# AgentCooper2002/AudioDiffuser

Measured on AMD Instinct MI355X. Metric: audio samples/sec (16384-sample waveform, 50-step Heun), higher is better.
Workload: dtype bf16; 1 GPU; BASELINE configs[1]: UNet1d 64 ch (c2), 16384-sample waveforms, KarrasSchedule N=50 heun, batch 64/GPU, random-init weights; global_batch=64, sampler=heun, num_steps=50, nfe=99, hipgraph=True, parallelism=batch-sharded x1, one all-gather

## Files before the change

### audiodiffuser_amd/_lib.py

```python
from __future__ import annotations

import ctypes as C
import os
from typing import Optional

from .config import UNet1dConfig

HERE = os.path.dirname(os.path.abspath(__file__))
LIB_PATH = os.environ.get("ADF_HIP_LIB") or os.path.join(HERE, "libadf_hip.so")
ADF_MAX_LAYERS = 12
DTYPE_F32, DTYPE_BF16, DTYPE_F32X3 = 0, 1, 2
FLAG_SEPARATE_GN_STATS = 1
SAMPLER_EDM, SAMPLER_EDM_ALPHA, SAMPLER_DPM_MULTISTEP, SAMPLER_DPM2, SAMPLER_ADPM2 = 0, 1, 2, 3, 4
SAMPLER_LMS, SAMPLER_DPM_SINGLESTEP, SAMPLER_DPM2M, SAMPLER_UNIPC, SAMPLER_ADPMPP2S = 5, 6, 7, 8, 9
SAMPLER_RF_EULER = 10


class AdfNetConfig(C.Structure):
    _fields_ = [
        ("channels", C.c_int32), ("num_filters", C.c_int32), ("window_length", C.c_int32), ("stride", C.c_int32),
        ("in_channels", C.c_int32), ("out_channels", C.c_int32),
        ("resnet_groups", C.c_int32), ("kernel_multiplier_downsample", C.c_int32),
        ("num_layers", C.c_int32),
        ("multipliers", C.c_int32 * (ADF_MAX_LAYERS + 1)),
        ("factors", C.c_int32 * ADF_MAX_LAYERS),
        ("num_blocks", C.c_int32 * ADF_MAX_LAYERS),
        ("attentions", C.c_int32 * ADF_MAX_LAYERS),
        ("attention_heads", C.c_int32), ("attention_multiplier", C.c_int32),
        ("use_skip_scale", C.c_int32), ("use_attention_bottleneck", C.c_int32),
        ("dtype", C.c_int32), ("flags", C.c_int32), ("num_classes", C.c_int32),
    ]


class AdfSamplerDesc(C.Structure):
    _fields_ = [
        ("kind", C.c_int32), ("num_steps", C.c_int32),
        ("s_tmin", C.c_float), ("s_tmax", C.c_float), ("s_churn", C.c_float), ("s_noise", C.c_float),
        ("use_heun", C.c_int32), ("alpha", C.c_float), ("order", C.c_int32), ("sigma_data", C.c_float),
        ("use_graph", C.c_int32), ("rho", C.c_float), ("eta", C.c_float), ("log_time_spacing", C.c_int32), ("eps_pred", C.c_int32),
        ("reflow", C.c_int32),
    ]


def make_sampler_desc(kind: int, num_steps: int, sigma_data: float, use_graph: bool, **fields) -> AdfSamplerDesc:
    unknown = set(fields) - {name for name, _ in AdfSamplerDesc._fields_}
    if unknown:
        raise TypeError(f"adf_sampler_desc has no field {sorted(unknown)}")
    return AdfSamplerDesc(kind=kind, num_steps=int(num_steps), sigma_data=sigma_data, use_graph=int(use_graph),
                          **{"s_noise": 1.0, "alpha": 1.0, **fields})


class AdfWaveNetConfig(C.Structure):
    _fields_ = [("residual_channels", C.c_int32), ("residual_layers", C.c_int32), ("dilation_cycle", C.c_int32),
                ("dim_in", C.c_int32), ("dim_mid", C.c_int32), ("dim_out", C.c_int32), ("dtype", C.c_int32)]


ADF_ADM_MAX_LEVELS = 8


class AdfAdmConfig(C.Structure):
    _fields_ = [("in_channels", C.c_int32), ("model_channels", C.c_int32), ("out_channels", C.c_int32), ("num_res_blocks", C.c_int32),
                ("n_mult", C.c_int32), ("channel_mult", C.c_int32 * ADF_ADM_MAX_LEVELS),
                ("n_attention_ds", C.c_int32), ("attention_ds", C.c_int32 * ADF_ADM_MAX_LEVELS),
                ("conv_resample", C.c_int32), ("num_heads", C.c_int32), ("num_head_channels", C.c_int32), ("use_scale_shift_norm", C.c_int32),
                ("resblock_updown", C.c_int32), ("use_new_attention_order", C.c_int32), ("num_classes", C.c_int32), ("dtype", C.c_int32)]


ADF_U2D_MAX_LEVELS, ADF_U2D_MAX_INIT_KERNELS = 8, 4


class AdfUNet2dConfig(C.Structure):
    _fields_ = [("ff_mult", C.c_double),
                ("dim", C.c_int32), ("cond_dim", C.c_int32), ("channels", C.c_int32), ("channels_out", C.c_int32), ("num_classes", C.c_int32),
                ("n_levels", C.c_int32), ("dim_mults", C.c_int32 * ADF_U2D_MAX_LEVELS),
                ("layer_attns", C.c_int32 * ADF_U2D_MAX_LEVELS), ("layer_cross_attns", C.c_int32 * ADF_U2D_MAX_LEVELS),
                ("num_resnet_blocks", C.c_int32), ("resnet_groups", C.c_int32), ("attn_heads", C.c_int32),
                ("layer_attns_depth", C.c_int32), ("layer_mid_attns_depth", C.c_int32), ("attend_at_middle", C.c_int32),
                ("n_init_kernels", C.c_int32), ("init_kernel_sizes", C.c_int32 * ADF_U2D_MAX_INIT_KERNELS),
                ("learned_sinu_pos_emb_dim", C.c_int32), ("num_time_tokens", C.c_int32),
                ("scale_skip_connection", C.c_int32), ("final_resnet_block", C.c_int32), ("dtype", C.c_int32)]


class AdfRunCounters(C.Structure):
    _fields_ = [("sampler_runs", C.c_int64), ("sampler_evals", C.c_int64), ("graph_captures", C.c_int64),
                ("graph_replays", C.c_int64), ("denoise_calls", C.c_int64), ("net_passes", C.c_int64)]


class AdfIstftConfig(C.Structure):
    _fields_ = [("n_fft", C.c_int32), ("hop_length", C.c_int32), ("center", C.c_int32), ("normalized", C.c_int32),
                ("spec_abs_exponent", C.c_double), ("spec_factor", C.c_double)]


FLAG_NEAREST_UPSAMPLE = 2
PRECOND_EDM, PRECOND_VE, PRECOND_VP, PRECOND_V_EDM = 0, 1, 2, 3
PRECOND_RF, PRECOND_RF_EDM = 4, 5
LOSS_X0_EDM, LOSS_X0_INV_SIGMA2, LOSS_RF = 0, 1, 2
LOSS_CHUNK = 4096
ABI_VERSION = 7

EXPORTS = {
    "adf_abi_version": (C.c_int, []),
    "adf_get_counters": (C.c_int, [C.c_void_p, C.POINTER(AdfRunCounters)]),
    "adf_create": (C.c_int, [C.POINTER(AdfNetConfig), C.POINTER(C.c_void_p)]),
    "adf_wavenet_create": (C.c_int, [C.POINTER(AdfWaveNetConfig), C.POINTER(C.c_void_p)]),
    "adf_adm_create": (C.c_int, [C.POINTER(AdfAdmConfig), C.POINTER(C.c_void_p)]),
    "adf_unet2d_create": (C.c_int, [C.POINTER(AdfUNet2dConfig), C.POINTER(C.c_void_p)]),
    "adf_set_image_shape": (C.c_int, [C.c_void_p, C.c_int, C.c_int]),
    "adf_set_dynamic_threshold": (C.c_int, [C.c_void_p, C.c_float]),
    "adf_set_preconditioning": (C.c_int, [C.c_void_p, C.c_int, C.c_double, C.c_double, C.c_double]),
    "adf_debug_coef_rows": (C.c_int, [C.c_void_p, C.c_void_p, C.c_int, C.POINTER(C.c_int), C.c_void_p]),
    "adf_destroy": (None, [C.c_void_p]),
    "adf_last_error": (C.c_char_p, [C.c_void_p]),
    "adf_num_weights": (C.c_int, [C.c_void_p]),
    "adf_weight_name": (C.c_char_p, [C.c_void_p, C.c_int]),
    "adf_weight_numel": (C.c_int64, [C.c_void_p, C.c_int]),
    "adf_load_weight": (C.c_int, [C.c_void_p, C.c_char_p, C.c_void_p, C.c_int64, C.c_void_p]),
    "adf_weights_missing": (C.c_int, [C.c_void_p]),
    "adf_set_condition": (C.c_int, [C.c_void_p, C.c_void_p, C.c_int, C.c_int, C.c_float, C.c_void_p]),
    "adf_net_forward": (C.c_int, [C.c_void_p, C.c_void_p, C.c_void_p, C.c_void_p, C.c_int, C.c_int, C.c_void_p]),
    "adf_denoise": (C.c_int, [C.c_void_p, C.c_void_p, C.c_void_p, C.c_float, C.c_float, C.c_void_p, C.c_int, C.c_int, C.c_void_p]),
    "adf_sampler_run": (C.c_int, [C.c_void_p, C.POINTER(AdfSamplerDesc), C.POINTER(C.c_float), C.c_int, C.c_void_p,
                                  C.c_void_p, C.c_int, C.c_void_p, C.c_int, C.c_int, C.c_void_p]),
    "adf_diffusion_loss": (C.c_int, [C.c_void_p, C.c_int, C.c_void_p, C.c_void_p, C.c_void_p, C.c_float, C.c_void_p, C.c_void_p, C.c_void_p,
                                     C.c_int, C.c_int, C.c_void_p]),
    "adf_loss_calls": (C.c_int64, [C.c_void_p]),
    "adf_sampler_nfe": (C.c_int, [C.POINTER(AdfSamplerDesc), C.POINTER(C.c_float), C.c_int]),
    "adf_debug_tap_shape": (C.c_int, [C.c_void_p, C.c_char_p, C.POINTER(C.c_int), C.POINTER(C.c_int)]),
    "adf_debug_tap_copy": (C.c_int, [C.c_void_p, C.c_char_p, C.c_void_p, C.c_void_p]),
    "adf_debug_tap_stats": (C.c_int, [C.c_void_p, C.c_char_p, C.c_void_p, C.POINTER(C.c_int), C.c_void_p]),
    "adf_debug_up_tile_plan": (C.c_int, [C.c_int, C.c_int, C.c_int, C.c_int, C.c_int, C.POINTER(C.c_int), C.POINTER(C.c_int), C.POINTER(C.c_int),
                                         C.POINTER(C.c_int)]),
    "adf_debug_dyn_threshold": (C.c_int, [C.c_void_p, C.c_void_p, C.c_int, C.c_longlong, C.c_float, C.c_void_p]),
    "adf_debug_tap_count": (C.c_int, [C.c_void_p]),
    "adf_debug_tap_name": (C.c_char_p, [C.c_void_p, C.c_int]),
    "adf_device_bytes": (C.c_int64, [C.c_void_p]),
    "adf_bench_resblock": (C.c_int, [C.c_void_p, C.c_int, C.c_int, C.c_int, C.c_int, C.POINTER(C.c_float), C.POINTER(C.c_float),
                                     C.POINTER(C.c_double), C.POINTER(C.c_double), C.POINTER(C.c_double), C.POINTER(C.c_double),
                                     C.c_void_p]),
    "adf_bench_layer": (C.c_int, [C.c_void_p, C.c_int, C.c_int, C.c_int, C.c_int, C.c_int, C.POINTER(C.c_float), C.POINTER(C.c_double),
                                  C.POINTER(C.c_double), C.POINTER(C.c_int), C.c_void_p]),
    "adf_bench_wavenet_layer": (C.c_int, [C.c_void_p, C.c_int, C.c_int, C.c_int, C.c_int, C.POINTER(C.c_float), C.POINTER(C.c_double),
                                          C.POINTER(C.c_double), C.c_void_p]),
    "adf_bench_loss_kernels": (C.c_int, [C.c_void_p, C.c_int, C.c_int, C.c_longlong, C.c_int, C.POINTER(C.c_float), C.POINTER(C.c_float),
                                         C.POINTER(C.c_double), C.POINTER(C.c_double), C.c_void_p]),
    "adf_istft_create": (C.c_int, [C.POINTER(AdfIstftConfig), C.c_void_p, C.POINTER(C.c_void_p)]),
    "adf_istft_basis": (C.c_int, [C.POINTER(AdfIstftConfig), C.c_void_p, C.c_void_p, C.c_void_p]),
    "adf_istft_run": (C.c_int, [C.c_void_p, C.c_void_p, C.c_int, C.c_int, C.c_void_p, C.c_int64, C.c_void_p]),
    "adf_istft_destroy": (None, [C.c_void_p]),
    "adf_stft_create": (C.c_int, [C.POINTER(AdfIstftConfig), C.c_void_p, C.POINTER(C.c_void_p)]),
    "adf_stft_basis": (C.c_int, [C.POINTER(AdfIstftConfig), C.c_void_p, C.c_void_p]),
    "adf_stft_run": (C.c_int, [C.c_void_p, C.c_void_p, C.c_int, C.c_int64, C.c_void_p, C.c_int, C.c_void_p]),
    "adf_stft_destroy": (None, [C.c_void_p]),
}

_lib: Optional[C.CDLL] = None


def load_library() -> C.CDLL:
    global _lib
    if _lib is not None:
        return _lib
    if not os.path.exists(LIB_PATH):
        raise RuntimeError(
            f"{LIB_PATH} is missing: build it with `python -m audiodiffuser_amd.build` "
            "(or __graft_entry__.build()). There is no CPU/PyTorch fallback for the HIP path.")
    lib = C.CDLL(LIB_PATH)
    for name, (res, args) in EXPORTS.items():
        fn = getattr(lib, name)
        fn.restype = res
        fn.argtypes = args
    got = lib.adf_abi_version()
    if got != ABI_VERSION:
        raise RuntimeError(f"{LIB_PATH} reports ABI version {got}, this binding was written against {ABI_VERSION}: rebuild the "
                           "library (python -m audiodiffuser_amd.build --force)")
    _lib = lib
    return lib


def make_config(cfg: UNet1dConfig, dtype: int, flags: int = 0) -> AdfNetConfig:
    cfg.validate()
    n = cfg.num_layers
    if n > ADF_MAX_LAYERS:
        raise ValueError("too many layers")
    c = AdfNetConfig()
    c.channels, c.num_filters, c.window_length, c.stride = cfg.channels, cfg.num_filters, cfg.window_length, cfg.stride
    c.in_channels, c.out_channels = cfg.in_channels, cfg.out_channels
    c.resnet_groups, c.kernel_multiplier_downsample = cfg.resnet_groups, cfg.kernel_multiplier_downsample
    c.num_layers = n
    for i, m in enumerate(cfg.multipliers):
        c.multipliers[i] = int(m)
    for i in range(n):
        c.factors[i] = int(cfg.factors[i])
        c.num_blocks[i] = int(cfg.num_blocks[i])
        c.attentions[i] = 1 if cfg.attentions[i] else 0
    c.attention_heads, c.attention_multiplier = cfg.attention_heads, cfg.attention_multiplier
    c.use_skip_scale = 1 if cfg.use_skip_scale else 0
    c.use_attention_bottleneck = 1 if cfg.use_attention_bottleneck else 0
    c.dtype, c.flags = dtype, flags | (FLAG_NEAREST_UPSAMPLE if cfg.use_nearest_upsample else 0)
    c.num_classes = int(cfg.num_classes) if cfg.class_cond else 0
    return c


def make_adm_config(cfg, dtype: int) -> AdfAdmConfig:
    c = AdfAdmConfig()
    c.in_channels, c.model_channels, c.out_channels, c.num_res_blocks = cfg.in_channels, cfg.model_channels, cfg.out_channels, cfg.num_res_blocks
    if len(cfg.channel_mult) > ADF_ADM_MAX_LEVELS or len(cfg.attention_ds) > ADF_ADM_MAX_LEVELS:
        raise ValueError("too many levels")
    c.n_mult = len(cfg.channel_mult)
    for i, m in enumerate(cfg.channel_mult):
        if int(m) != m:
            raise ValueError("channel_mult entries must be integers")
        c.channel_mult[i] = int(m)
    c.n_attention_ds = len(cfg.attention_ds)
    for i, d in enumerate(cfg.attention_ds):
        c.attention_ds[i] = int(d)
    c.conv_resample, c.num_heads, c.num_head_channels = int(cfg.conv_resample), cfg.num_heads, cfg.num_head_channels
    c.use_scale_shift_norm, c.resblock_updown = int(cfg.use_scale_shift_norm), int(cfg.resblock_updown)
    c.use_new_attention_order = int(cfg.use_new_attention_order)
    c.num_classes = int(cfg.num_classes) if cfg.num_classes is not None else 0
    c.dtype = dtype
    return c


def make_unet2d_config(cfg, dtype: int) -> AdfUNet2dConfig:
    n = len(cfg.dim_mults)
    if n > ADF_U2D_MAX_LEVELS or len(cfg.init_cross_embed_kernel_sizes) > ADF_U2D_MAX_INIT_KERNELS:
        raise ValueError("too many levels / cross-embed kernel sizes")
    c = AdfUNet2dConfig()
    c.ff_mult = float(cfg.ff_mult)
    c.dim, c.cond_dim, c.channels, c.channels_out, c.num_classes = cfg.dim, cfg.cdim, cfg.channels, cfg.out_channels, int(cfg.num_classes)
    c.n_levels = n
    for i in range(n):
        c.dim_mults[i], c.layer_attns[i], c.layer_cross_attns[i] = int(cfg.dim_mults[i]), int(cfg.layer_attns[i]), int(cfg.layer_cross_attns[i])
    c.num_resnet_blocks, c.resnet_groups, c.attn_heads = cfg.num_resnet_blocks, cfg.resnet_groups, cfg.attn_heads
    c.layer_attns_depth, c.layer_mid_attns_depth, c.attend_at_middle = cfg.layer_attns_depth, cfg.layer_mid_attns_depth, int(cfg.attend_at_middle)
    ks = sorted(cfg.init_cross_embed_kernel_sizes)
    c.n_init_kernels = len(ks)
    for i, k in enumerate(ks):
        c.init_kernel_sizes[i] = int(k)
    c.learned_sinu_pos_emb_dim, c.num_time_tokens = cfg.learned_sinu_pos_emb_dim, cfg.num_time_tokens
    c.scale_skip_connection, c.final_resnet_block = int(cfg.scale_skip_connection), int(cfg.final_resnet_block)
    c.dtype = dtype
    return c


def make_wavenet_config(cfg, dtype: int) -> AdfWaveNetConfig:
    c = AdfWaveNetConfig()
    c.residual_channels, c.residual_layers, c.dilation_cycle = cfg.residual_channels, cfg.residual_layers, cfg.dilation_cycle
    c.dim_in, c.dim_mid, c.dim_out = cfg.dim_in, cfg.dim_mid, cfg.dim_out
    c.dtype = dtype
    return c


class AdfError(RuntimeError):
    pass


def check(lib: C.CDLL, handle, rc: int, what: str) -> None:
    if rc != 0:
        msg = lib.adf_last_error(handle)
        raise AdfError(f"{what}: {msg.decode() if msg else 'unknown error'}")
```

### audiodiffuser_amd/csrc/adf_gemm.h

```cpp
#pragma once
#include "adf_common.h"

namespace adf {

constexpr int kARows = 144;
constexpr int kTapGroup = 3;

struct GemmSeg {
    const void* src0;
    const void* src1;
    int c0, c1;
    const float* ab;
    GnFinalizeArgs gn;
    float scale1;
    int act;
    int taps, stride, off0, step;
    const void* w;
    const void* wfrag;
    int nchunk;
};

struct GemmArgs {
    GemmSeg seg[2];
    int nseg;
    int B, lin, mrows, n, n_pad;
    int gn_ready;
    int flat;
    int seg_rows;
    const float* bias0;
    const float* bias1;
    int bias_mod;
    const void* res;
    int gelu;
    void* out;
    int out_rows, out_c;
    int scatter_f, scatter_pad;
    int phase_c;
    double* stats;
    int stats_groups;
};

template <int N>
__device__ __forceinline__ void gemm_bias_load(const GemmArgs& a, const int (&bi)[N], const bool (&ok)[N], float (&out)[N]) {
    const bool h0 = a.bias0 != nullptr, h1 = a.bias1 != nullptr;
    const float* const dmy = (const float*)a.seg[0].w;
    const float* const p0 = h0 ? a.bias0 : dmy;
    const float* const p1 = h1 ? a.bias1 : dmy;
    float v0[N], v1[N];
#pragma unroll
    for (int k = 0; k < N; ++k) {
        const int idx = ok[k] ? bi[k] : 0;
        v0[k] = p0[h0 ? idx : 0]; v1[k] = p1[h1 ? idx : 0];
    }
#pragma unroll
    for (int k = 0; k < N; ++k) out[k] = ok[k] ? (h0 ? v0[k] : 0.f) + (h1 ? v1[k] : 0.f) : 0.f;
}

typedef __attribute__((ext_vector_type(8))) __bf16 bf16x8_t;
typedef __attribute__((ext_vector_type(16))) float f32x16_t;
typedef __attribute__((ext_vector_type(4))) float f32x4_t;
typedef __attribute__((ext_vector_type(2))) float f32x2_t;


constexpr int kLdsPitch = 144;
__device__ __forceinline__ int lds_swz(int row, int c16) { return row * kLdsPitch + (c16 << 4); }

#define ADF_GLOAD16(dst, ptr) asm volatile("global_load_dwordx4 %0, %1, off" : "=v"(dst) : "v"(ptr) : "memory")

__device__ __forceinline__ const char* uniform_ptr(const void* p) {
    const unsigned long long v = (unsigned long long)p;
    const unsigned lo = __builtin_amdgcn_readfirstlane((unsigned)v);
    const unsigned hi = __builtin_amdgcn_readfirstlane((unsigned)(v >> 32));
    return (const char*)(((unsigned long long)hi << 32) | lo);
}

template <int TM, int TN>
constexpr int gemm_lds_bytes() {
    constexpr int main_b = kARows * kLdsPitch + kTapGroup * TN * kLdsPitch;
    constexpr int epi_b = TM * TN * 4;
    return main_b > epi_b ? main_b : epi_b;
}

template <int TAPS, int MT, int NT, typename FA, typename FW>
__device__ __forceinline__ void mfma_chunk_bf16(f32x16_t (&acc)[MT][NT], int h, FA addrA, FW addrW) {
    constexpr int NS = TAPS * 4;
    bf16x8_t fa[2][MT], fb[2][NT];
#pragma unroll
    for (int i = 0; i < MT; ++i) fa[0][i] = *(const bf16x8_t*)addrA(0, i, h);
#pragma unroll
    for (int j = 0; j < NT; ++j) fb[0][j] = *(const bf16x8_t*)addrW(0, j, h);
#pragma unroll
    for (int st = 0; st < NS; ++st) {
        const int cur = st & 1, nxt = cur ^ 1;
        if (st + 1 < NS) {
            const int tap = (st + 1) >> 2, ks = (st + 1) & 3;
#pragma unroll
            for (int i = 0; i < MT; ++i) fa[nxt][i] = *(const bf16x8_t*)addrA(tap, i, ks * 2 + h);
#pragma unroll
            for (int j = 0; j < NT; ++j) fb[nxt][j] = *(const bf16x8_t*)addrW(tap, j, ks * 2 + h);
        }
        __builtin_amdgcn_sched_barrier(0);
#pragma unroll
        for (int i = 0; i < MT; ++i)
#pragma unroll
            for (int j = 0; j < NT; ++j)
                acc[i][j] = __builtin_amdgcn_mfma_f32_32x32x16_bf16(fa[cur][i], fb[cur][j], acc[i][j], 0, 0, 0);
        __builtin_amdgcn_sched_barrier(0);
    }
}

template <typename T, int MT, int NT, int WM, int WN>
__global__ void __launch_bounds__(64 * WM * WN) conv_gemm_kernel(const GemmArgs a) {
    constexpr int TM = 32 * MT * WM, TN = 32 * NT * WN, NTHR = 64 * WM * WN;
    constexpr int EPC = Elem<T>::kPerChunk;
    constexpr int KC = kRowBytes / (int)sizeof(T);
    constexpr int A_CH = (kARows * 8 + NTHR - 1) / NTHR;
    constexpr int W_CH = (kTapGroup * TN * 8 + NTHR - 1) / NTHR;
    constexpr bool kBf16 = sizeof(T) == 2;
    constexpr bool kX3 = IsX3<T>::value;
    extern __shared__ __attribute__((aligned(16))) char smem[];
    char* ldsA = smem;
    char* ldsW = smem + kARows * kLdsPitch;

    const int tid = threadIdx.x, lane = tid & 63, wave = tid >> 6;
    const int r = lane & 31, h = lane >> 5;
    const int wm = wave / WN, wn = wave % WN;
    const int tiles_n = (a.n_pad + TN - 1) / TN;
    int bid = blockIdx.x;
    const int tn_i = bid % tiles_n; bid /= tiles_n;
    const int seg = a.flat ? a.seg_rows : TM;
    const int nsegs = TM / seg;
    int b0, m0;
    long long R0;
    if (a.flat) {
        R0 = (long long)bid * TM;
        b0 = (int)(R0 / a.mrows);
        m0 = 0;
    } else {
        const int tiles_m = (a.mrows + TM - 1) / TM;
        const int tm_i = bid % tiles_m;
        b0 = bid / tiles_m;
        m0 = tm_i * TM;
        R0 = (long long)b0 * a.mrows + m0;
    }
    const int n0 = tn_i * TN;
    const int c16 = tid & 7;

    f32x16_t acc[MT][NT];
#pragma unroll
    for (int i = 0; i < MT; ++i)
#pragma unroll
        for (int j = 0; j < NT; ++j)
#pragma unroll
            for (int e = 0; e < 16; ++e) acc[i][j][e] = 0.f;

    const int ntg0 = (a.seg[0].taps + kTapGroup - 1) / kTapGroup;
    const int nit0 = a.seg[0].nchunk * ntg0;
    const int ntg1 = a.nseg > 1 ? (a.seg[1].taps + kTapGroup - 1) / kTapGroup : 1;
    const int nit = nit0 + (a.nseg > 1 ? a.seg[1].nchunk * ntg1 : 0);

    u32x4_t ra[A_CH];
    u32x4_t rw[W_CH];
    f32x4_t abq[EPC / 2];
    float raw_scale = 1.0f;
    unsigned avalid = 0;

    const int wrow0 = tid >> 3;
    int arow_idx[A_CH];
    auto setup_segment = [&](const GemmSeg& sg) {
        const int off_min = sg.step > 0 ? sg.off0 : sg.off0 - (sg.taps - 1);
        const int segrows = (seg - 1) * sg.stride + sg.taps;
        const int nrows = nsegs * segrows;
        const int p_lo = m0 * sg.stride + off_min;
#pragma unroll
        for (int i = 0; i < A_CH; ++i) {
            const int row = (tid + i * NTHR) >> 3;
            const int j = a.flat ? row / segrows : 0;
            const int p = p_lo + (row - j * segrows);
            const int bb = b0 + j;
            const bool ok = row < nrows && p >= 0 && p < a.lin && bb < a.B;
            arow_idx[i] = ok ? bb * a.lin + p : -1;
        }
    };
    auto load_regs = [&](int it) {
        const bool s1 = it >= nit0;
        const GemmSeg& sg = s1 ? a.seg[1] : a.seg[0];
        const int local = s1 ? it - nit0 : it;
        const int ntg = s1 ? ntg1 : ntg0;
        const int chunk = local / ntg, tg = local - chunk * ntg;
        if (local == 0) setup_segment(sg);
        if (tg == 0) {
            const int ctot = sg.c0 + sg.c1;
            const int cidx = chunk * KC + c16 * EPC;
            const bool cvalid = cidx < ctot;
            const bool from1 = sg.c1 > 0 && cidx >= sg.c0;
            const char* src0u = uniform_ptr(sg.src0);
            const char* src1u = uniform_ptr(sg.src1);
            const char* src = from1 ? src1u : src0u;
            const int c0u = __builtin_amdgcn_readfirstlane(sg.c0), c1u = __builtin_amdgcn_readfirstlane(sg.c1);
            const unsigned rowbytes = (unsigned)(from1 ? c1u : c0u) * (unsigned)sizeof(T);
            const unsigned colbytes = (unsigned)(from1 ? cidx - c0u : cidx) * (unsigned)sizeof(T);
            avalid = 0;
#pragma unroll
            for (int i = 0; i < A_CH; ++i) {
                const bool ok = cvalid && arow_idx[i] >= 0;
                const unsigned off = ok ? (unsigned)arow_idx[i] * rowbytes + colbytes : 0u;
                ra[i] = *(const u32x4_t*)(src + off);
                avalid |= (ok ? 1u : 0u) << i;
            }
            const float* abp = sg.ab ? sg.ab + (cvalid ? (unsigned)(b0 * ctot + cidx) * 2u : 0u) : (const float*)sg.w;
#pragma unroll
            for (int e = 0; e < EPC / 2; ++e) abq[e] = *(const f32x4_t*)(abp + e * 4);
            raw_scale = from1 ? sg.scale1 : 1.0f;
        }
        const char* wp = (const char*)sg.w + (size_t)(chunk * sg.taps + tg * kTapGroup) * a.n_pad * kRowBytes;
#pragma unroll
        for (int i = 0; i < W_CH; ++i) {
            const int row = wrow0 + i * (NTHR / 8);
            const int tap_l = row / TN, n_l = row - tap_l * TN;
            const unsigned woff = (unsigned)((tap_l * a.n_pad + n0 + n_l) * kRowBytes + c16 * 16);
            rw[i] = *(const u32x4_t*)(wp + woff);
        }
    };

    const int lds_row0 = tid >> 3;
    auto store_lds = [&](int it) {
        const bool s1 = it >= nit0;
        const GemmSeg& sg = s1 ? a.seg[1] : a.seg[0];
        const int local = s1 ? it - nit0 : it;
        const int ntg = s1 ? ntg1 : ntg0;
        const int tg = local % ntg;
        if (tg == 0) {
            const int nrows = nsegs * ((seg - 1) * sg.stride + sg.taps);
            const bool act = sg.act != 0;
            const bool use_ab = sg.ab != nullptr;
            f32x2_t fa2[EPC / 2], fb2[EPC / 2];
#pragma unroll
            for (int e = 0; e < EPC / 2; ++e) {
                fa2[e] = use_ab ? f32x2_t{abq[e].x, abq[e].z} : f32x2_t{raw_scale, raw_scale};
                fb2[e] = use_ab ? f32x2_t{abq[e].y, abq[e].w} : f32x2_t{0.f, 0.f};
            }
#pragma unroll
            for (int i = 0; i < A_CH; ++i) {
                const int row = lds_row0 + i * (NTHR / 8);
                if (row < nrows) {
                    u32x4_t q = u32x4_t{0u, 0u, 0u, 0u};
                    if ((avalid >> i) & 1u) {
                        float f[EPC];
                        unpack16<T>(ra[i], f);
                        if (act) {
#pragma unroll
                            for (int e = 0; e < EPC / 2; ++e) {
                                const f32x2_t x2 = {f[2 * e], f[2 * e + 1]};
                                const f32x2_t v2 = x2 * fa2[e] + fb2[e];
                                const f32x2_t z2 = v2 * -1.4426950408889634f;
                                f32x2_t d2 = {__builtin_amdgcn_exp2f(z2.x), __builtin_amdgcn_exp2f(z2.y)};
                                d2 = d2 + 1.0f;
                                const f32x2_t r2 = {__builtin_amdgcn_rcpf(d2.x), __builtin_amdgcn_rcpf(d2.y)};
                                const f32x2_t y2 = v2 * r2;
                                f[2 * e] = y2.x; f[2 * e + 1] = y2.y;
                            }
                        } else {
#pragma unroll
                            for (int e = 0; e < EPC / 2; ++e) {
                                const f32x2_t x2 = {f[2 * e], f[2 * e + 1]};
                                const f32x2_t v2 = x2 * fa2[e] + fb2[e];
                                f[2 * e] = v2.x; f[2 * e + 1] = v2.y;
                            }
                        }
                        q = pack16<T>(f);
                    }
                    if constexpr (kX3) {
                        float f4[4];
                        unpack16<float>(q, f4);
                        u32x2_t hi, lo;
                        split_bf16x4(f4, hi, lo);
                        *(u32x2_t*)(ldsA + lds_swz(row, c16 >> 1) + (c16 & 1) * 8) = hi;
                        *(u32x2_t*)(ldsA + lds_swz(row, 4 + (c16 >> 1)) + (c16 & 1) * 8) = lo;
                    } else {
                        *(u32x4_t*)(ldsA + lds_swz(row, c16)) = q;
                    }
                }
            }
        }
#pragma unroll
        for (int i = 0; i < W_CH; ++i) {
            const int row = lds_row0 + i * (NTHR / 8);
            if (row < kTapGroup * TN) *(u32x4_t*)(ldsW + lds_swz(row, c16)) = rw[i];
        }
    };

    auto compute = [&](int it) {
        const bool s1 = it >= nit0;
        const GemmSeg& sg = s1 ? a.seg[1] : a.seg[0];
        const int local = s1 ? it - nit0 : it;
        const int ntg = s1 ? ntg1 : ntg0;
        const int tg = local % ntg;
        const int off_min = sg.step > 0 ? sg.off0 : sg.off0 - (sg.taps - 1);
        const int segrows = (seg - 1) * sg.stride + sg.taps;
        int ntap = sg.taps - tg * kTapGroup;
        ntap = ntap > kTapGroup ? kTapGroup : ntap;
        int abase[MT];
#pragma unroll
        for (int i = 0; i < MT; ++i) {
            const int ti = (wm * MT + i) * 32 + r;
            const int j = a.flat ? ti / seg : 0;
            abase[i] = j * segrows + (ti - j * seg) * sg.stride;
        }
        for (int tap_l = 0; tap_l < ntap; ++tap_l) {
            const int aoff = sg.off0 + (tg * kTapGroup + tap_l) * sg.step - off_min;
            int arow[MT], wrow[NT];
#pragma unroll
            for (int i = 0; i < MT; ++i) arow[i] = abase[i] + aoff;
#pragma unroll
            for (int j = 0; j < NT; ++j) wrow[j] = tap_l * TN + (wn * NT + j) * 32 + r;
            if constexpr (kBf16) {
#pragma unroll
                for (int ks = 0; ks < 4; ++ks) {
                    bf16x8_t fa_[MT], fb_[NT];
#pragma unroll
                    for (int i = 0; i < MT; ++i) fa_[i] = *(const bf16x8_t*)(ldsA + lds_swz(arow[i], ks * 2 + h));
#pragma unroll
                    for (int j = 0; j < NT; ++j) fb_[j] = *(const bf16x8_t*)(ldsW + lds_swz(wrow[j], ks * 2 + h));
// ... 944 lines not shown
```

### audiodiffuser_amd/csrc/adf_gemm.hip

```cpp
#include "adf_gemm.h"
#include "adf_gemm_pp.h"
#include "adf_gemm_rb.h"
#include "adf_gemm_rbx3.h"
#include "adf_gemm_up.h"
#include "adf_kernels.h"
#include <cstdio>
#include <cstdlib>
#include <cstring>
#include <vector>


#ifdef ADF_RB_STAMP
namespace adf { __device__ unsigned long long adf_rb_stamps[8 * 16]; }
extern "C" int adf_debug_rb_stamps(unsigned long long* out) {
    return (int)hipMemcpyFromSymbol(out, HIP_SYMBOL(adf::adf_rb_stamps), sizeof(unsigned long long) * 8 * 16);
}
#endif

#ifdef ADF_RB_TL
namespace adf { __device__ unsigned adf_rb_tl[2 * 8 * 128]; }
extern "C" int adf_debug_rb_timeline(unsigned* out) {
    return (int)hipMemcpyFromSymbol(out, HIP_SYMBOL(adf::adf_rb_tl), sizeof(unsigned) * 2 * 8 * 128);
}
#endif

#ifdef ADF_UP_TL
namespace adf { __device__ unsigned long long adf_up_tl[2 * 8 * kUpTlWave]; }
extern "C" int adf_debug_up_timeline(unsigned long long* out) {
    return (int)hipMemcpyFromSymbol(out, HIP_SYMBOL(adf::adf_up_tl), sizeof(unsigned long long) * 2 * 8 * adf::kUpTlWave);
}
#endif

namespace adf {

namespace {

template <typename T, int MT, int NT, int WM, int WN>
const char* launch_variant(const GemmArgs& a, hipStream_t stream) {
    constexpr int TM = 32 * MT * WM, TN = 32 * NT * WN, NTHR = 64 * WM * WN;
    constexpr int lds = gemm_lds_bytes<TM, TN>();
    if (!raise_lds_limit<lds, conv_gemm_kernel<T, MT, NT, WM, WN>>()) return "hipFuncSetAttribute(MaxDynamicSharedMemorySize) failed";
    const int tiles_n = (a.n_pad + TN - 1) / TN;
    const long long tiles_m = a.flat ? ((long long)a.B * a.mrows + TM - 1) / TM : (long long)((a.mrows + TM - 1) / TM) * a.B;
    const long long blocks = (long long)tiles_n * tiles_m;
    if (blocks <= 0 || blocks > 0x7fffffffLL) return "conv_gemm: bad grid";
    hipLaunchKernelGGL((conv_gemm_kernel<T, MT, NT, WM, WN>), dim3((unsigned)blocks), dim3(NTHR), lds, stream, a);
    return hipGetLastError() == hipSuccess ? nullptr : "conv_gemm: launch failed";
}

int ws_lds_bytes(const GemmArgs& a, int tn) {
    long long wrows = 0;
    for (int s = 0; s < a.nseg; ++s) wrows += (long long)a.seg[s].nchunk * a.seg[s].taps * tn;
    const long long b = wrows * kLdsPitch + 2LL * kWsARows * kLdsPitch + kWsScratch;
    return b > 0x7fffffff ? 0x7fffffff : (int)b;
}

template <typename T, int NT, int WN>
const char* launch_ws_variant(const GemmArgs& a, hipStream_t stream) {
    constexpr int TN = NT * WN * 32;
    if (!raise_lds_limit<160 * 1024, conv_gemm_ws_kernel<T, NT, WN>>()) return "hipFuncSetAttribute(MaxDynamicSharedMemorySize, ws) failed";
    const int tiles_n = (a.n_pad + TN - 1) / TN;
    const long long tiles_m_total = (long long)((a.mrows + 127) / 128) * a.B;
    if (tiles_m_total <= 0 || tiles_m_total > 0x7fffffffLL) return "conv_gemm_ws: bad tile count";
    long long bpn = device_cus() / tiles_n;
    if (bpn < 1) bpn = 1;
    if (bpn > tiles_m_total) bpn = tiles_m_total;
    hipLaunchKernelGGL((conv_gemm_ws_kernel<T, NT, WN>), dim3((unsigned)(bpn * tiles_n)), dim3(512), (size_t)ws_lds_bytes(a, TN), stream, a, (int)tiles_m_total,
                       (int)bpn);
    return hipGetLastError() == hipSuccess ? nullptr : "conv_gemm_ws: launch failed";
}

template <int CIN, int COUT, int F, int MTP>
const char* launch_up_mt(const GemmArgs& a, const UpTilePlan& tp, hipStream_t stream) {
    typedef UpCfg<CIN, COUT, F, MTP> Cfg;
    if (!raise_lds_limit<160 * 1024, conv_gemm_up_kernel<CIN, COUT, F, MTP>>()) return "hipFuncSetAttribute(MaxDynamicSharedMemorySize, up) failed";
    static_assert(Cfg::kLds <= 160 * 1024, "up kernel LDS budget");
    if (tp.tile_rows != Cfg::TM || tp.items <= 0 || tp.items > 0x7fffffffLL) return "conv_gemm_up: bad tile count";
    const long long grid = tp.items < kUpGrid ? tp.items : kUpGrid;
    hipLaunchKernelGGL((conv_gemm_up_kernel<CIN, COUT, F, MTP>), dim3((unsigned)grid), dim3(512), Cfg::kLds, stream, a, (int)tp.items, tp.tiles_per_sample);
    return hipGetLastError() == hipSuccess ? nullptr : "conv_gemm_up: launch failed";
}
template <int CIN, int COUT, int F>
const char* launch_up(const GemmArgs& a, hipStream_t stream) {
    typedef UpCfg<CIN, COUT, F, 1> C1;
    if (a.lin < 1) return "conv_gemm_up: bad tile count";
    const UpTilePlan tp = up_tile_plan(a.B, a.lin, C1::WROWS, C1::NPASS);
    if (tp.mt == 1) return launch_up_mt<CIN, COUT, F, 1>(a, tp, stream);
    if (tp.mt == 2) return launch_up_mt<CIN, COUT, F, 2>(a, tp, stream);
    return launch_up_mt<CIN, COUT, F, 4>(a, tp, stream);
}

template <int MT>
const char* launch_pp(const GemmArgs& a, hipStream_t stream) {
    if (!raise_lds_limit<kPpLds, conv_gemm_pp_kernel<MT>>()) return "hipFuncSetAttribute(MaxDynamicSharedMemorySize, pp) failed";
    constexpr int TM = 128 * MT;
    const int tiles_m = a.mrows / TM, tiles_n = a.n_pad / kPpTN;
    int tm_shift = 0;
    while ((1 << tm_shift) < tiles_m) ++tm_shift;
    const long long tiles_total = (long long)a.B * tiles_m * tiles_n;
    if (tiles_total <= 0 || tiles_total > (1 << 22)) return "conv_gemm_pp: bad tile count";
    const long long grid = tiles_total < device_cus() ? tiles_total : device_cus();
    hipLaunchKernelGGL(conv_gemm_pp_kernel<MT>, dim3((unsigned)grid), dim3(512), kPpLds, stream, a, (int)tiles_total, tm_shift, tiles_n);
    return hipGetLastError() == hipSuccess ? nullptr : "conv_gemm_pp: launch failed";
}

bool stats_groups_ok(int channels, int groups, int lo, int hi) {
    const int gs = groups > 0 ? channels / groups : 0;
    return gs > 0 && gs * groups == channels && (gs & (gs - 1)) == 0 && gs >= lo && gs <= hi;
}
bool pow2(int v) { return v > 0 && (v & (v - 1)) == 0; }

struct RbForm {
    int esz;
    int blk_ch;
    int max_blk;
    bool even_pairs;
    bool wide_n;
};
constexpr RbForm kRbBf16 = {2, 64, kRbMaxBlk, true, true}, kRbX3 = {4, 32, kRbx3MaxBlk, false, false};

bool rb_raw0(const GemmArgs& a) { return !a.seg[0].gn.gamma && !a.seg[0].ab && !a.seg[0].act && a.seg[0].c1 == 0; }

bool rb_shape_ok(const GemmArgs& a, const RbForm& f, bool with_stats) {
    const GemmSeg& g0 = a.seg[0];
    if (a.scatter_f || a.gelu || a.mrows % 128 || a.lin != a.mrows || a.out_rows != a.mrows) return false;
    if (a.n != a.n_pad || a.out_c != a.n || (a.n != 128 && a.n != 256) || a.bias_mod != a.n) return false;
    if (!pow2(a.mrows / 128)) return false;
    const bool raw0 = rb_raw0(a);
    if (!raw0 && (!g0.gn.gamma || !g0.act)) return false;
    if (g0.taps != 3 || g0.off0 != -1 || g0.stride != 1 || g0.step != 1) return false;
    auto seg_ok = [&](int c0, int c1, int nb_before) {
        if (c0 % 64 || c1 % 64 || nb_before + (c0 + c1) / f.blk_ch > f.max_blk) return false;
        return !(f.even_pairs && ((c0 + c1) / 64) % 2);
    };
    if (!seg_ok(g0.c0, g0.c1, 0)) return false;
    if (!raw0 && g0.c0 + g0.c1 > kPpMaxCin) return false;
    if (!raw0) {
        const GnFinalizeArgs& gn = g0.gn;
        if (gn.G < 1 || (gn.c0 + gn.c1) % gn.G || gn.c0 % gn.G || gn.c1 % gn.G) return false;
        const int gs = (gn.c0 + gn.c1) / gn.G;
        if (gn.c0 % gs) return false;
        for (int cs : {gn.c0, gn.c1}) {
            if (cs == 0) continue;
            const int fg = cs / gn.G;
            if (gs != fg && gs != 2 * fg) return false;
        }
    }
    if (raw0 && (a.nseg > 1 || a.res)) return false;
    if (a.res && a.nseg > 1) return false;
    if (a.nseg > 1) {
        const GemmSeg& g1 = a.seg[1];
        if (g1.taps != 1 || g1.off0 != 0 || g1.stride != 1 || g1.step != 1 || g1.ab || g1.act) return false;
        if (!seg_ok(g1.c0, g1.c1, (g0.c0 + g0.c1) / f.blk_ch)) return false;
    }
    if (a.phase_c && (!raw0 || (a.phase_c & (a.phase_c - 1)) || a.phase_c < 64 || a.n % a.phase_c)) return false;
    return !(with_stats && a.stats) || stats_groups_ok(a.phase_c ? a.phase_c : a.out_c, a.stats_groups, 8, 64);
}

struct RbTiles { int tm, nh; long long total; };
bool rb_tiles(const GemmArgs& a, const RbForm& f, long long min_tiles, RbTiles& t) {
    t = RbTiles{256, 1, 0};
    auto at = [&](int tm) -> long long {
        if (a.mrows % tm || !pow2(a.mrows / tm)) return 0;
        const long long tiles_m = (long long)a.B * (a.mrows / tm);
        t.tm = tm;
        t.nh = (f.wide_n && a.n == 256 && tiles_m >= min_tiles) ? 2 : 1;
        return tiles_m * (a.n / (kPpTN * t.nh));
    };
    t.total = at(256);
    if (t.total < min_tiles) t.total = at(128);
    return t.total <= (1 << 22) && t.total >= min_tiles;
}

template <typename ArgsT>
void rb_fill_args(const GemmArgs& a, const RbForm& f, const RbTiles& t, ArgsT& r) {
    const GemmSeg& g0 = a.seg[0];
    memset(&r, 0, sizeof(r));
    int nb = 0;
    auto add_seg = [&](const void* s0, const void* s1, int c0, int c1, const void* w, int taps, bool table, float scale1) {
        for (int c = 0; c < c0 + c1; c += f.blk_ch, ++nb) {
            const bool from1 = c >= c0;
            RbBlk& e = r.blk[nb];
            e.src = (const char*)(from1 ? s1 : s0) + (size_t)(from1 ? c - c0 : c) * f.esz;
            e.pitch = (unsigned)(from1 ? c1 : c0) * (unsigned)f.esz;
            e.w = (const char*)w + (size_t)(c / f.blk_ch) * taps * a.n_pad * kRowBytes;
            e.tab = table ? c * 8 : -1;
            e.scale = from1 ? scale1 : 1.0f;
        }
    };
    add_seg(g0.src0, g0.src1, g0.c0, g0.c1, g0.w, 3, !rb_raw0(a), 1.0f);
    r.h.nb3 = nb;
    if (a.nseg > 1) add_seg(a.seg[1].src0, a.seg[1].src1, a.seg[1].c0, a.seg[1].c1, a.seg[1].w, 1, false, a.seg[1].scale1);
    r.h.res = a.nseg == 1 ? a.res : nullptr;
    r.h.nb1 = nb - r.h.nb3;
    r.h.B = a.B; r.h.L = a.mrows;
    r.h.n = a.n;
    r.h.gn = g0.gn;
    r.h.bias0 = a.bias0; r.h.bias1 = a.bias1;
    r.h.out = a.out;
    if (a.stats) {
        r.h.stats = a.stats; r.h.stats_groups = a.stats_groups;
        r.h.stats_mod = a.phase_c;
    }
    r.h.tiles_n = a.n / (kPpTN * t.nh);
    while ((1 << r.h.tm_shift) < a.mrows / t.tm) ++r.h.tm_shift;
    r.h.tiles_total = (int)t.total;
}

const char* launch_rb(const GemmArgs& a, long long min_tiles, hipStream_t stream) {
    RbTiles t;
    RbArgs r;
    rb_tiles(a, kRbBf16, min_tiles, t);
    rb_fill_args(a, kRbBf16, t, r);
    if (!raise_lds_limit<kRbLds, conv_gemm_rb_kernel<1, false, 2>, conv_gemm_rb_kernel<2, false, 2>, conv_gemm_rb_kernel<1, true, 2>, conv_gemm_rb_kernel<2, true, 2>,
                         conv_gemm_rb_kernel<1, false, 1>, conv_gemm_rb_kernel<2, false, 1>, conv_gemm_rb_kernel<1, true, 1>, conv_gemm_rb_kernel<2, true, 1>>())
        return "hipFuncSetAttribute(MaxDynamicSharedMemorySize, rb) failed";
    const long long grid = t.total < device_cus() ? t.total : device_cus();
    const bool raw0 = rb_raw0(a);
    auto go = [&](auto kern) { hipLaunchKernelGGL(kern, dim3((unsigned)grid), dim3(512), kRbLds, stream, r); };
    if (t.tm == 256) {
        if (t.nh == 2 && raw0) go(conv_gemm_rb_kernel<2, true, 2>);
        else if (t.nh == 2) go(conv_gemm_rb_kernel<2, false, 2>);
        else if (raw0) go(conv_gemm_rb_kernel<1, true, 2>);
        else go(conv_gemm_rb_kernel<1, false, 2>);
    } else {
        if (t.nh == 2 && raw0) go(conv_gemm_rb_kernel<2, true, 1>);
        else if (t.nh == 2) go(conv_gemm_rb_kernel<2, false, 1>);
        else if (raw0) go(conv_gemm_rb_kernel<1, true, 1>);
        else go(conv_gemm_rb_kernel<1, false, 1>);
    }
    return hipGetLastError() == hipSuccess ? nullptr : "conv_gemm_rb: launch failed";
}

const char* launch_rbx3(const GemmArgs& a, long long min_tiles, hipStream_t stream) {
    RbTiles t;
    Rbx3Args r;
    rb_tiles(a, kRbX3, min_tiles, t);
    rb_fill_args(a, kRbX3, t, r);
    if (!raise_lds_limit<kRbLds, conv_gemm_rbx3_kernel<2>, conv_gemm_rbx3_kernel<1>>()) return "hipFuncSetAttribute(MaxDynamicSharedMemorySize, rbx3) failed";
    const long long grid = t.total < device_cus() ? t.total : device_cus();
    if (t.tm == 256) hipLaunchKernelGGL(conv_gemm_rbx3_kernel<2>, dim3((unsigned)grid), dim3(512), kRbLds, stream, r);
    else hipLaunchKernelGGL(conv_gemm_rbx3_kernel<1>, dim3((unsigned)grid), dim3(512), kRbLds, stream, r);
    return hipGetLastError() == hipSuccess ? nullptr : "conv_gemm_rbx3: launch failed";
}

bool pp_eligible(const GemmArgs& a, int tm) {
    if (a.scatter_f || a.mrows % tm || a.lin != a.mrows || a.out_rows != a.mrows) return false;
    if (a.n != a.n_pad || a.out_c != a.n || a.n_pad % kPpTN || a.n_pad > kPpMaxN) return false;
    if (!pow2(a.mrows / tm)) return false;
    if (a.res && a.nseg > 1) return false;
    int nb = a.res ? a.n / 64 : 0;
    for (int s = 0; s < a.nseg; ++s) {
        const GemmSeg& g = a.seg[s];
        if (g.stride != 1 || g.step != 1) return false;
        if (!((g.taps == 3 && g.off0 == -1) || (g.taps == 1 && g.off0 == 0))) return false;
        if (g.c0 % 64 || g.c1 % 64 || (g.ab && g.c0 + g.c1 > kPpMaxCin)) return false;
        if (s == 1 && (g.ab || g.act)) return false;
        nb += (g.c0 + g.c1) / 64;
    }
    return nb >= 2;
}

const void* pp_identity(int n, hipStream_t stream, const char** err) {
    static void* cache_dev[kMaxDevices][kPpMaxN / 64 + 1] = {};
    void** cache = cache_dev[current_device()];
    const int idx = n / 64;
    if (cache[idx]) return cache[idx];
    const size_t elems = (size_t)(n / 64 + kTapGroup) * n * 64;
    std::vector<uint16_t> hbuf(elems, 0);
    for (int r = 0; r < n; ++r) hbuf[((size_t)(r / 64) * n + r) * 64 + (r % 64)] = 0x3F80;
    void* d = nullptr;
    if (hipMalloc(&d, elems * 2) != hipSuccess) { *err = "conv_gemm_pp: hipMalloc(identity) failed"; return nullptr; }
    if (hipMemcpyAsync(d, hbuf.data(), elems * 2, hipMemcpyHostToDevice, stream) != hipSuccess || hipStreamSynchronize(stream) != hipSuccess) {
        *err = "conv_gemm_pp: identity upload failed";
        return nullptr;
    }
    cache[idx] = d;
    return d;
}

template <typename T, int MT, int NT>
const char* launch_ksplit(const GemmArgs& a, hipStream_t stream) {
    constexpr int lds = 4 * ks_wave_lds(MT, NT);
    constexpr int TM = 32 * MT, TN = 32 * NT;
    if (!raise_lds_limit<lds, conv_gemm_ksplit_kernel<T, MT, NT>>()) return "hipFuncSetAttribute(MaxDynamicSharedMemorySize, ksplit) failed";
    const int tiles_n = (a.n_pad + TN - 1) / TN;
    const long long tiles_m = a.flat ? ((long long)a.B * a.mrows + TM - 1) / TM : (long long)((a.mrows + TM - 1) / TM) * a.B;
    const long long blocks = tiles_m * tiles_n;
    if (blocks <= 0 || blocks > 0x7fffffffLL) return "conv_gemm_ksplit: bad grid";
    hipLaunchKernelGGL((conv_gemm_ksplit_kernel<T, MT, NT>), dim3((unsigned)blocks), dim3(256), lds, stream, a);
    return hipGetLastError() == hipSuccess ? nullptr : "conv_gemm_ksplit: launch failed";
}

template <typename T>
const char* dispatch(const GemmArgs& a, int tm, int tn, hipStream_t s) {
    if (tm == 128 && tn == 128) return launch_variant<T, 2, 2, 2, 2>(a, s);
    if (tm == 128 && tn == 64) return launch_variant<T, 2, 1, 2, 2>(a, s);
    if (tm == 128 && tn == 32) return launch_variant<T, 1, 1, 4, 1>(a, s);
    if (tm == 64 && tn == 128) return launch_variant<T, 1, 2, 2, 2>(a, s);
    if (tm == 64 && tn == 64) return launch_variant<T, 1, 1, 2, 2>(a, s);
    if (tm == 64 && tn == 32) return launch_variant<T, 1, 1, 2, 1>(a, s);
    if (tm == 32 && tn == 128) return launch_variant<T, 1, 1, 1, 4>(a, s);
    if (tm == 32 && tn == 64) return launch_variant<T, 1, 1, 1, 2>(a, s);
    return launch_variant<T, 1, 1, 1, 1>(a, s);
}

struct GemmSwitches {
    int trace = adf_route_switch("ADF_GEMM_TRACE", 0);
    int up = adf_route_switch("ADF_GEMM_UP", 1);
    int pp = adf_route_switch("ADF_GEMM_PP", 1);
    int ws = adf_route_switch("ADF_GEMM_WS", 1);
    long long rb_min_tiles = min_tiles_of(adf_route_switch("ADF_GEMM_RB", 1));
    long long rbx3_min_tiles = min_tiles_of(adf_route_switch("ADF_GEMM_RBX3", 1));
    int gn_in_kernel = (int)adf_tuning("ADF_GEMM_GN", 1);
    int min_blocks = (int)adf_tuning("ADF_GEMM_MINBLOCKS", 512);
    int ksplit = (int)adf_tuning("ADF_GEMM_KSPLIT", 1);
    long long ksplit_rows = adf_tuning("ADF_GEMM_KSPLIT_ROWS", 4096);
    int ksplit_minit = (int)adf_tuning("ADF_GEMM_KSPLIT_MINIT", 4);
    long long ws_min_m = adf_tuning("ADF_GEMM_WS_MINM", 256);
    static long long min_tiles_of(int sw) { return sw == 0 ? -1 : (sw >= 2 ? 32 : 256); }
};
const GemmSwitches& switches() {
    static const GemmSwitches s;
    return s;
}

enum class Route { refused, up, ksplit, rbx3, rb, pp, ws, plain };
const char* const kRouteName[] = {"", "up", "ksplit", "rbx3", "rb", "pp", "ws", "plain"};

struct GemmPlan {
    Route route = Route::refused;
    const char* refusal = nullptr;
    int tm = 0, tn = 0;
    int flat = 0, seg_rows = 0;
    bool stats = false;
    bool stats_traced = false;
    bool gn_in_kernel = false;
    int up_cfg = 0;
    bool ident_seg = false;
};

bool rb_takes(const GemmArgs& a, bool x3, bool with_stats) {
    const long long min_tiles = x3 ? switches().rbx3_min_tiles : switches().rb_min_tiles;
    const RbForm& f = x3 ? kRbX3 : kRbBf16;
    RbTiles t;
    return min_tiles >= 0 && rb_shape_ok(a, f, with_stats) && rb_tiles(a, f, min_tiles, t);
}

GemmPlan decide_conv_gemm(const GemmArgs& a, int dtype) {
    const GemmSwitches& sw = switches();
    const bool dtype_bf16 = dtype == 1, x3 = dtype == 2;
    GemmPlan p;
    auto refuse = [&](const char* why) { p.refusal = why; return p; };
    auto take_rb = [&](bool stats) {
        p.route = x3 ? Route::rbx3 : Route::rb;
        p.tm = 256; p.tn = 128;
        p.stats = stats;
        p.gn_in_kernel = true;
        return p;
    };
    if (a.phase_c) {
        const char* const no = "conv_gemm: a 3-tap-form transposed conv that conv_gemm_rb_kernel does not take";
        if (dtype == 0 || a.flat) return refuse(no);
        const bool with_stats = a.stats && rb_takes(a, x3, true);
        if (!with_stats && !rb_takes(a, x3, false)) return refuse(no);
        p.stats_traced = with_stats;
        return take_rb(with_stats);
    }
    if (a.nseg < 1 || a.nseg > 2) return refuse("conv_gemm: nseg must be 1 or 2");
    if (a.n_pad % 32) return refuse("conv_gemm: n_pad must be a multiple of 32");
    const int epc = dtype_bf16 ? 8 : 4;
    if (a.n % epc || a.out_c % epc) return refuse("conv_gemm: output channels must be a multiple of a 16-byte chunk");
    const long long esz = dtype_bf16 ? 2 : 4;
    if ((long long)a.B * a.out_rows * a.out_c * esz >= (1LL << 32)) return refuse("conv_gemm: output tensor must be < 4 GiB");
    bool raw = true;
    for (int s = 0; s < a.nseg; ++s) {
        const GemmSeg& g = a.seg[s];
        if (g.c0 % epc || g.c1 % epc) return refuse("conv_gemm: channel counts must be multiples of a 16-byte chunk");
        if (g.step != 1 && g.step != -1) return refuse("conv_gemm: step must be +-1");
        if (g.taps < 1 || g.stride < 1) return refuse("conv_gemm: bad taps/stride");
        if (g.ab) raw = false;
        if ((long long)a.B * a.lin * (g.c0 > g.c1 ? g.c0 : g.c1) * esz >= (1LL << 32)) return refuse("conv_gemm: input tensor must be < 4 GiB");
    }
    const bool can_flat = raw && !a.scatter_f && a.lin == a.mrows && (a.mrows & (a.mrows - 1)) == 0;
    int tm = 0, flat = 0;
    for (int cand = 128; cand >= 32 && !tm; cand >>= 1) {
        if (can_flat && a.mrows < cand) {
            bool fits = true;
            for (int s = 0; s < a.nseg; ++s)
                if ((cand / a.mrows) * ((a.mrows - 1) * a.seg[s].stride + a.seg[s].taps) > kARows) fits = false;
            if (fits) { tm = cand; flat = 1; continue; }
        }
        bool fits = true;
        for (int s = 0; s < a.nseg; ++s)
            if ((cand - 1) * a.seg[s].stride + a.seg[s].taps > kARows) fits = false;
        if (!fits) continue;
        if (cand > 32 && a.mrows <= cand / 2) continue;
        tm = cand;
    }
    if (!tm) return refuse("conv_gemm: no tile shape fits (stride/taps too large)");
    int tn = a.n_pad >= 128 ? 128 : (a.n_pad >= 64 ? 64 : 32);
    if (a.n_pad % tn && a.n_pad % 64 == 0) tn = 64;
    auto nblocks = [&](int tm_, int tn_) {
        const long long tmn = flat ? ((long long)a.B * a.mrows + tm_ - 1) / tm_ : (long long)((a.mrows + tm_ - 1) / tm_) * a.B;
        return tmn * ((a.n_pad + tn_ - 1) / tn_);
    };
    while (nblocks(tm, tn) < sw.min_blocks && tn > 32) tn >>= 1;
    while (nblocks(tm, tn) < sw.min_blocks && tm > 32) {
        tm >>= 1;
        if (flat && a.mrows >= tm) flat = 0;
    }
    p.route = Route::plain;
    p.tm = tm; p.tn = tn;
    p.flat = flat;
    p.seg_rows = flat ? a.mrows : tm;
    if (a.stats) {
        const int nthr = (tm == 64 && tn == 32) || (tm == 32 && tn == 64) ? 128 : ((tm == 32 && tn == 32) ? 64 : 256);
        const int rpk = nthr * epc / tn;
        p.stats = stats_groups_ok(a.out_c, a.stats_groups, epc, tn) && (!flat || a.mrows % rpk == 0);
    }
    p.stats_traced = p.stats;
    auto take = [&](Route r, int tm_, int tn_, bool stats) {
        p.route = r;
        p.tm = tm_; p.tn = tn_;
        p.stats = p.stats_traced = stats;
        return p;
    };
    const GemmSeg& g0 = a.seg[0];
    const bool gn_pending = g0.gn.gamma != nullptr;
    {
        const int f = a.scatter_f, cout = a.out_c, cin = g0.c0;
        if (sw.up && dtype_bf16 && (f == 2 || f == 4) && a.nseg == 1 && g0.taps == 2 && g0.stride == 1 && g0.off0 == 0 && g0.step == -1 && !g0.ab &&
            !gn_pending && !g0.act && g0.scale1 == 1.0f && g0.wfrag && g0.c1 == 0 && a.n == f * cout && a.n == a.n_pad && a.mrows == a.lin + 1 &&
            a.out_rows == a.lin * f && a.scatter_pad == f / 2 && a.bias_mod == cout && !a.res && !a.gelu && !a.bias1 &&
            (!a.stats || a.stats_groups == 8)) {
            if (cin == 256 && cout == 256 && f == 4) p.up_cfg = 1;
            else if (cin == 256 && cout == 128 && f == 2) p.up_cfg = 2;
            else if (sw.up >= 2 && cin == 128 && cout == 128 && f == 2) p.up_cfg = 3;
            else if (sw.up >= 2 && cin == 128 && cout == 64 && f == 2) p.up_cfg = 4;
            if (p.up_cfg) return take(Route::up, 64, 256, a.stats != nullptr);
        }
    }
    {
        int nit_total = 0;
        bool ks_ok = sw.ksplit && !a.scatter_f && (long long)a.B * a.mrows <= sw.ksplit_rows;
        const int ks_flat = (can_flat && a.mrows < 32 && 32 % a.mrows == 0) ? 1 : 0;
        const int ks_seg = ks_flat ? a.mrows : 32;
        if (!ks_flat && !raw && a.mrows < 32) ks_ok = false;
        for (int s = 0; s < a.nseg; ++s) {
            const GemmSeg& g = a.seg[s];
            if (g.stride != 1 || g.taps > kTapGroup) ks_ok = false;
            if ((32 / ks_seg) * ((ks_seg - 1) + g.taps) > ks_a_rows(1)) ks_ok = false;
            nit_total += g.nchunk;
        }
        if (ks_ok && nit_total >= sw.ksplit_minit) {
            const bool big = sw.ksplit != 32 && !ks_flat && a.mrows % 64 == 0 && a.n_pad % 64 == 0 &&
                             (long long)a.B * (a.mrows / 64) * (a.n_pad / 64) >= 128;
            const int tile = big ? 64 : 32;
            p.flat = ks_flat;
            p.seg_rows = big ? 64 : ks_seg;
            const int rows_per_wave = 64 / (tile / epc);
            return take(Route::ksplit, tile, tile, a.stats && stats_groups_ok(a.out_c, a.stats_groups, epc, tile) && p.seg_rows % rows_per_wave == 0);
        }
    }
    const bool rb_raw = !gn_pending && !g0.ab && !g0.act && a.nseg == 1 && !a.res && g0.taps == 3;
    if (dtype != 0 && !flat && ((gn_pending && sw.gn_in_kernel && !a.gn_ready) || rb_raw) && rb_takes(a, x3, true)) return take_rb(a.stats != nullptr);
    if (sw.pp && dtype_bf16 && !flat && tm == 128 && !(g0.taps == 1 && a.nseg == 1) && (sw.pp == 2 || !a.res)) {
        const long long t256 = pp_eligible(a, 256) ? (long long)a.B * (a.mrows / 256) * (a.n_pad / kPpTN) : 0;
        const long long t128 = pp_eligible(a, 128) ? (long long)a.B * (a.mrows / 128) * (a.n_pad / kPpTN) : 0;
        const long long need = sw.pp >= 2 ? 128 : 256;
        const int ptm = t256 >= need ? 256 : ((t128 >= need && sw.pp != 3) ? 128 : 0);
        if (ptm) {
            p.ident_seg = a.res != nullptr;
            const int gn_gs = g0.gn.G > 0 ? (g0.gn.c0 + g0.gn.c1) / g0.gn.G : 0;
            p.gn_in_kernel = g0.taps == 3 && sw.gn_in_kernel && gn_gs > 0 && g0.gn.c0 % gn_gs == 0;
            return take(Route::pp, ptm, 128, a.stats && stats_groups_ok(a.out_c, a.stats_groups, 8, 64));
        }
    }
    {
        bool ws_ok = sw.ws && !x3 && !flat && tm == 128 && a.n_pad >= 64;
        for (int s = 0; s < a.nseg; ++s)
            if (a.seg[s].stride != 1 || 127 + a.seg[s].taps > kWsARows) ws_ok = false;
        const long long tiles_m_total = (long long)((a.mrows + 127) / 128) * a.B;
        if (ws_ok && tiles_m_total >= sw.ws_min_m) {
            int wtn = 0;
            if (a.n_pad >= 128 && ws_lds_bytes(a, 128) <= 160 * 1024) wtn = 128;
            else if (sw.ws == 64 && ws_lds_bytes(a, 64) <= 160 * 1024) wtn = 64;
            if (wtn) return take(Route::ws, 128, wtn, a.stats && stats_groups_ok(a.out_c, a.stats_groups, epc, wtn / 2));
        }
    }
    return p;
}

}

bool conv_gemm_phase_eligible(const GemmArgs& a, int dtype, bool* stats_fused) {
    const GemmPlan p = decide_conv_gemm(a, dtype);
    if (stats_fused) *stats_fused = p.stats;
    return a.phase_c && p.route != Route::refused;
}

const char* launch_conv_gemm(const GemmArgs& a_in, int dtype, hipStream_t stream, bool* stats_fused) {
    const GemmSwitches& sw = switches();
    const GemmPlan p = decide_conv_gemm(a_in, dtype);
    if (stats_fused) *stats_fused = p.stats;
    if (p.route == Route::refused) return p.refusal;
    GemmArgs a = a_in;
    a.flat = p.flat;
    a.seg_rows = p.seg_rows;
    if (!p.stats) a.stats = nullptr;
    if (a.nseg > 1) a.seg[1].gn.gamma = nullptr;
    if (p.ident_seg) {
        const char* err = nullptr;
        const void* ident = pp_identity(a.n, stream, &err);
        if (!ident) return err;
        GemmSeg& g = a.seg[1];
        g = GemmSeg{};
        g.src0 = a.res; g.src1 = nullptr; g.c0 = a.n; g.c1 = 0; g.ab = nullptr; g.scale1 = 1.0f; g.act = 0;
        g.taps = 1; g.stride = 1; g.off0 = 0; g.step = 1; g.w = ident; g.nchunk = a.n / 64;
        a.nseg = 2;
        a.res = nullptr;
    }
    if (a.seg[0].gn.gamma && !p.gn_in_kernel) {
        const char* err = a.gn_ready ? nullptr : launch_gn_finalize(a.seg[0].gn, stream);
        a.seg[0].gn.gamma = nullptr;
        if (err) return err;
    }
    if (sw.trace) {
        fprintf(stderr, "[adf gemm] %-6s B=%d lin=%d mrows=%d n=%d/%d nseg=%d seg0(c=%d+%d taps=%d stride=%d off0=%d step=%d ab=%d act=%d)", kRouteName[(int)p.route], a.B,
                a.lin, a.mrows, a.n, a.n_pad, a.nseg, a.seg[0].c0, a.seg[0].c1, a.seg[0].taps, a.seg[0].stride, a.seg[0].off0, a.seg[0].step, a.seg[0].ab != nullptr,
                a.seg[0].act);
        if (a.nseg > 1) fprintf(stderr, " seg1(c=%d+%d taps=%d ab=%d)", a.seg[1].c0, a.seg[1].c1, a.seg[1].taps, a.seg[1].ab != nullptr);
        fprintf(stderr, " res=%d gelu=%d scatter=%d out=%dx%d stats=%d flat=%d tile=%dx%d\n", a.res != nullptr, a.gelu, a.scatter_f, a.out_rows, a.out_c, p.stats_traced,
                a.flat, p.tm, p.tn);
    }
    switch (p.route) {
    case Route::up:
        if (p.up_cfg == 1) return launch_up<256, 256, 4>(a, stream);
        if (p.up_cfg == 2) return launch_up<256, 128, 2>(a, stream);
        if (p.up_cfg == 3) return launch_up<128, 128, 2>(a, stream);
        return launch_up<128, 64, 2>(a, stream);
    case Route::ksplit:
        if (p.tm == 64) return dtype == 1 ? launch_ksplit<bf16_t, 2, 2>(a, stream) : (dtype == 2 ? launch_ksplit<f32x3_t, 2, 2>(a, stream) : launch_ksplit<float, 2, 2>(a, stream));
        return dtype == 1 ? launch_ksplit<bf16_t, 1, 1>(a, stream) : (dtype == 2 ? launch_ksplit<f32x3_t, 1, 1>(a, stream) : launch_ksplit<float, 1, 1>(a, stream));
    case Route::rbx3: return launch_rbx3(a, sw.rbx3_min_tiles, stream);
    case Route::rb: return launch_rb(a, sw.rb_min_tiles, stream);
    case Route::pp: return p.tm == 256 ? launch_pp<2>(a, stream) : launch_pp<1>(a, stream);
    case Route::ws:
        if (p.tn == 128) return dtype == 1 ? launch_ws_variant<bf16_t, 2, 2>(a, stream) : launch_ws_variant<float, 2, 2>(a, stream);
        return dtype == 1 ? launch_ws_variant<bf16_t, 1, 2>(a, stream) : launch_ws_variant<float, 1, 2>(a, stream);
    default: return dtype == 1 ? dispatch<bf16_t>(a, p.tm, p.tn, stream) : (dtype == 2 ? dispatch<f32x3_t>(a, p.tm, p.tn, stream) : dispatch<float>(a, p.tm, p.tn, stream));
    }
}

}

extern "C" int adf_debug_up_tile_plan(int cin, int cout, int f, int B, int L, int* tile_rows, int* items, int* rounds, int* dead_rows) {
    using namespace adf;
    if (B < 1 || L < 1 || (long long)B * L > 0x3fffffffLL) return 1;
    UpTilePlan tp;
    if (cin == 256 && cout == 256 && f == 4) tp = up_tile_plan(B, L, UpCfg<256, 256, 4, 1>::WROWS, UpCfg<256, 256, 4, 1>::NPASS);
    else if (cin == 256 && cout == 128 && f == 2) tp = up_tile_plan(B, L, UpCfg<256, 128, 2, 1>::WROWS, UpCfg<256, 128, 2, 1>::NPASS);
    else if (cin == 128 && cout == 128 && f == 2) tp = up_tile_plan(B, L, UpCfg<128, 128, 2, 1>::WROWS, UpCfg<128, 128, 2, 1>::NPASS);
    else if (cin == 128 && cout == 64 && f == 2) tp = up_tile_plan(B, L, UpCfg<128, 64, 2, 1>::WROWS, UpCfg<128, 64, 2, 1>::NPASS);
    else return 1;
    if (tile_rows) *tile_rows = tp.tile_rows;
    if (items) *items = (int)tp.items;
    if (rounds) *rounds = (int)tp.rounds;
    if (dead_rows) *dead_rows = tp.dead_rows;
    return 0;
}
```

### audiodiffuser_amd/csrc/adf_gemm_rb.h

```cpp
#pragma once
#include "adf_gemm.h"
#include "adf_gemm_pp.h"
#include <type_traits>

namespace adf {

#ifdef ADF_RB_STAMP
extern __device__ unsigned long long adf_rb_stamps[8 * 16];
#endif

#ifdef ADF_RB_TL
extern __device__ unsigned adf_rb_tl[2 * 8 * 128];
constexpr int kRbLds = kPpLds + 3072;
#else
constexpr int kRbLds = kPpLds;
#endif
constexpr int kRbMaxBlk = 24;
#ifndef ADF_RB_KNOCK
#define ADF_RB_KNOCK 0
#endif
#ifndef ADF_RB_DOT2
#define ADF_RB_DOT2 1
#endif
#ifndef ADF_RB_NT
#define ADF_RB_NT 0
#endif
#ifndef ADF_RB_W3
#define ADF_RB_W3 1
#endif
#ifndef ADF_RB_PRIO
#define ADF_RB_PRIO 4
#endif
#ifndef ADF_RB_FILL2
#define ADF_RB_FILL2 1
#endif
#ifndef ADF_RB_PRESLAB
#define ADF_RB_PRESLAB 1
#endif


struct RbBlk {
    const char* src;
    const char* w;
    unsigned pitch;
    int tab;
    float scale;
    int pad_;
};

struct RbHead {
    int nb3, nb1;
    int B, L;
    int tm_shift;
    int tiles_n;
    int tiles_total;
    int n;
    GnFinalizeArgs gn;
    const float* bias0; const float* bias1;
    void* out;
    const void* res;
    double* stats; int stats_groups;
    int stats_mod;
};
struct RbArgs {
    RbHead h;
    RbBlk blk[kRbMaxBlk];
};

__device__ __forceinline__ void rb_dma2(const char* base, unsigned va, unsigned vb, unsigned la, unsigned lb) {
    asm volatile("s_mov_b32 m0, %3\n\ts_nop 0\n\tglobal_load_lds_dwordx4 %1, %0\n\t"
                 "s_mov_b32 m0, %4\n\ts_nop 0\n\tglobal_load_lds_dwordx4 %2, %0"
                 :: "s"(base), "v"(va), "v"(vb), "s"(la), "s"(lb) : "memory");
}
__device__ __forceinline__ void rb_dma1(const char* base, unsigned va, unsigned la) {
    asm volatile("s_mov_b32 m0, %2\n\ts_nop 0\n\tglobal_load_lds_dwordx4 %1, %0" :: "s"(base), "v"(va), "s"(la) : "memory");
}

template <int I, int N, typename F>
__device__ __forceinline__ void rb_static_for(F&& f) {
    if constexpr (I < N) {
        f(std::integral_constant<int, I>{});
        rb_static_for<I + 1, N>(f);
    }
}

template <int NH, bool RAW, int MH = 2>
__global__ void __launch_bounds__(512) conv_gemm_rb_kernel(const RbArgs a) {
    typedef bf16_t T;
    constexpr int TM = 128 * MH, HP = TM / 8;
    constexpr int TNB = kPpTN * NH;
    constexpr bool W3 = ADF_RB_W3 == 2 || (ADF_RB_W3 == 1 && (MH == 1 || NH == 2)) || (ADF_RB_W3 == 3 && MH == 1) || (ADF_RB_W3 == 4 && (MH == 1 || NH == 1));
    extern __shared__ __attribute__((aligned(16))) char smem[];
    const RbHead H = a.h;
    const RbBlk e_first[3] = {a.blk[0], a.blk[1], a.blk[2]};
    asm volatile("" :: "s"(H.nb3), "s"(H.tiles_total), "s"(H.gn.stats0), "s"(H.gn.gamma), "s"(H.gn.film), "s"(H.bias0), "s"(H.out), "s"(H.stats),
                 "s"(e_first[0].src), "s"(e_first[1].src), "s"(e_first[2].src), "s"(e_first[0].tab), "s"(e_first[1].tab), "s"(e_first[2].tab));
    char* const ldsScr = smem + kPpOffScr;
    char* const ldsTab = smem + kPpOffTab;
    float* const ldsBias = (float*)(smem + kPpOffBias);

    const int tid = threadIdx.x, lane = tid & 63;
    const int wave = __builtin_amdgcn_readfirstlane(tid >> 6);
    const int r = lane & 31, h = lane >> 5;
    const int wm = wave >> 1, wn = wave & 1;
    const int lrow = lane >> 3;
    const int chunk = (lane & 7) ^ ((((wave & 1) << 2) + (lane >> 4)) & 7);
    const int srow = wave * 8 + lrow;
    const unsigned lane_lds = (unsigned)lane * 16u;

    if (ADF_RB_PRIO == 4) __builtin_amdgcn_s_setprio(3);
    if (ADF_RB_PRIO == 1 && wave >= 4) __builtin_amdgcn_s_setprio(1);
    if (ADF_RB_PRIO == 3 && wave >= 4) __builtin_amdgcn_s_setprio(2);
    const int nblk_grid = (int)gridDim.x, bidx = (int)blockIdx.x;
    const int t_lo = (int)((unsigned)bidx * (unsigned)H.tiles_total / (unsigned)nblk_grid);
    const int t_hi = (int)((unsigned)(bidx + 1) * (unsigned)H.tiles_total / (unsigned)nblk_grid);
    const int ntiles = t_hi - t_lo;
    if (ntiles <= 0) return;
    const int nb3 = H.nb3, nb1 = H.nb1, nb = nb3 + nb1;
    const int ctot0 = H.gn.c0 + H.gn.c1;
    const int tn_shift = H.tiles_n > 1 ? 1 : 0;
    const int tm_mask = (1 << H.tm_shift) - 1;

    struct Tile { int b0, m0, n0; };
    auto tile_of = [&](int tseq) __attribute__((always_inline)) -> Tile {
        const int t = t_lo + tseq;
        const int tml = t >> tn_shift;
        Tile g;
        g.n0 = (t & (H.tiles_n - 1)) * TNB;
        g.b0 = tml >> H.tm_shift;
        g.m0 = (tml & tm_mask) * TM;
        return g;
    };
    const int b_first = tile_of(0).b0;

    struct Blk {
        const char* abase;
        const char* w;
        unsigned pitch;
        int tab;
        float scale;
        int edge;
        int taps;
    };
    int d_t = 0, d_k = 0;
    Tile d_tile = tile_of(0);
    auto make_desc_of = [&](const RbBlk& e) __attribute__((always_inline)) -> Blk {
        Blk d;
        const int three = d_k < nb3;
        const int p_lo = d_tile.m0 - three;
        d.pitch = e.pitch;
        d.abase = e.src + (long long)(d_tile.b0 * H.L + p_lo) * (long long)e.pitch;
        d.w = e.w + (unsigned)d_tile.n0 * (unsigned)kRowBytes;
        d.tab = e.tab >= 0 ? ((d_tile.b0 - b_first) & 1) * kPpTab + e.tab : -1;
        d.scale = e.scale;
        d.taps = three ? 3 : 1;
        d.edge = three ? ((d_tile.m0 == 0 ? 1 : 0) | (d_tile.m0 + TM >= H.L ? 2 : 0)) : 0;
        return d;
    };
    auto make_desc = [&]() __attribute__((always_inline)) -> Blk { return make_desc_of(a.blk[d_k]); };
    auto advance = [&]() __attribute__((always_inline)) {
        if (++d_k == nb) {
            d_k = 0;
            if (++d_t < ntiles) d_tile = tile_of(d_t);
        }
    };
    const unsigned slab = (unsigned)H.n * (unsigned)kRowBytes;

    const unsigned colbytes = (unsigned)chunk * 16u;
    auto issue_a01 = [&](const Blk& d, unsigned st) __attribute__((always_inline)) {
        if (ADF_RB_KNOCK & 2) return;
        const unsigned v = (unsigned)srow * d.pitch + colbytes;
        const unsigned v0 = ((d.edge & 1) && srow == 0) ? v + d.pitch : v;
        const unsigned l = st + (unsigned)wave * 1024u;
        rb_dma2(d.abase, v0, v + 64u * d.pitch, l, l + 8192u);
    };
    auto issue_a23 = [&](const Blk& d, unsigned st) __attribute__((always_inline)) {
        if ((ADF_RB_KNOCK & 2) || MH == 1) return;
        const unsigned v = (unsigned)(srow + 128) * d.pitch + colbytes;
        const unsigned l = st + (unsigned)wave * 1024u + 16384u;
        rb_dma2(d.abase, v, v + 64u * d.pitch, l, l + 8192u);
    };
    auto issue_halo = [&](const Blk& d, unsigned st) __attribute__((always_inline)) {
        if (ADF_RB_KNOCK & 2) return;
        if (wave == 0 && d.taps == 3) {
            const unsigned vh = (unsigned)TM * d.pitch + ((d.edge & 2) ? 0u : (unsigned)lrow * d.pitch) + colbytes;
            if (lane < 16) rb_dma1(d.abase, vh, st + (unsigned)HP * 1024u);
        }
    };
    const unsigned wlane = (unsigned)srow * (unsigned)kRowBytes + colbytes;
    auto issue_w = [&](const char* wsrc, int wst) __attribute__((always_inline)) {
        if (ADF_RB_KNOCK & 4) return;
        const unsigned l = (unsigned)(kPpOffW + wst * kPpWStage) + (unsigned)wave * 1024u;
        rb_dma2(wsrc, wlane, wlane + 64u * (unsigned)kRowBytes, l, l + 8192u);
    };
    auto issue_w_at = [&](const char* wsrc, unsigned wofs) __attribute__((always_inline)) {
        if (ADF_RB_KNOCK & 4) return;
        const unsigned l = (unsigned)kPpOffW + wofs + (unsigned)wave * 1024u;
        rb_dma2(wsrc, wlane, wlane + 64u * (unsigned)kRowBytes, l, l + 8192u);
    };

    struct GnLoaded { double s0, q0, s1, q1; float gamma, beta, f1s, f1h, f2s, f2h; };
    auto gn_two = [&](int c) __attribute__((always_inline)) -> bool {
        const GnFinalizeArgs& g = H.gn;
        const int ctot = g.c0 + g.c1, gs = ctot / g.G;
        const bool from1 = (c / gs) * gs >= g.c0;
        return gs > (from1 ? g.c1 : g.c0) / g.G;
    };
    auto gn_load = [&](int b, int c) __attribute__((always_inline)) -> GnLoaded {
        const GnFinalizeArgs& g = H.gn;
        const int ctot = g.c0 + g.c1;
        const int gs = ctot / g.G;
        const int cstart = (c / gs) * gs;
        const bool from1 = cstart >= g.c0;
        const double* st = gn_select_ptr(from1, g.stats0, g.stats1);
        const int csrc = from1 ? g.c1 : g.c0;
        const int lc = from1 ? cstart - g.c0 : cstart;
        const int fg = csrc / g.G;
        const int g0 = lc / fg;
        const bool two = gs > fg;
        const double* p0 = st + ((size_t)b * g.G + g0) * 2;
        const double* p1 = two ? p0 + 2 : p0;
        const bool hf = g.film != nullptr, hf2 = hf && g.film2 != nullptr;
        int cd = c;
        asm volatile("" : "+v"(cd));
        const float* const f1 = hf ? g.film + (size_t)b * g.film_bstride : g.gamma;
        const float* const f2 = hf2 ? g.film2 + (size_t)b * g.film2_bstride : g.gamma;
        GnLoaded r;
        r.s0 = p0[0]; r.q0 = p0[1]; r.s1 = p1[0]; r.q1 = p1[1];
        r.gamma = g.gamma[c]; r.beta = g.beta[c];
        r.f1s = f1[cd]; r.f1h = f1[hf ? ctot + cd : cd]; r.f2s = f2[cd]; r.f2h = f2[hf2 ? ctot + cd : cd];
        return r;
    };
    auto gn_store = [&](int c, const GnLoaded& v, int slot) __attribute__((always_inline)) {
        const bool two = gn_two(c);
        const bool hf = H.gn.film != nullptr, hf2 = hf && H.gn.film2 != nullptr;
        GnRaw r;
        r.sum = v.s0 + (two ? v.s1 : 0.0); r.sq = v.q0 + (two ? v.q1 : 0.0);
        r.gamma = v.gamma; r.beta = v.beta;
        r.fs = hf ? v.f1s + 1.0f + (hf2 ? v.f2s : 0.f) : 1.0f;
        r.fh = hf ? v.f1h + (hf2 ? v.f2h : 0.f) : 0.0f;
        float A, Bc;
        gn_affine_finish<true>(H.gn, c, r, A, Bc);
        *(f32x2_t*)(ldsTab + slot * kPpTab + c * 8) = f32x2_t{A, Bc};
    };
    auto fill_table = [&](int b, int slot) __attribute__((always_inline)) {
        int t1 = tid;
        asm volatile("" : "+v"(t1));
        const GnLoaded v = gn_load(b, t1 < ctot0 ? t1 : ctot0 - 1);
        if (t1 < ctot0) gn_store(t1, v, slot);
    };

    auto silu4 = [&](const u32x2_t& raw, const float* fa, const float* fb, bool act) __attribute__((always_inline)) -> u32x2_t {
        float v[4], ex[4];
        const float ec = act ? -1.4426950408889634f : 0.0f, ed = act ? 0.0f : -200.0f;
        v[0] = __uint_as_float(raw.x << 16); v[1] = __uint_as_float(raw.x & 0xffff0000u);
        v[2] = __uint_as_float(raw.y << 16); v[3] = __uint_as_float(raw.y & 0xffff0000u);
#pragma unroll
        for (int e = 0; e < 4; ++e) v[e] = fmaf(v[e], fa[e], fb[e]);
#pragma unroll
        for (int e = 0; e < 4; ++e) ex[e] = __builtin_amdgcn_exp2f(fmaf(v[e], ec, ed));
#pragma unroll
        for (int e = 0; e < 4; ++e) ex[e] = __builtin_amdgcn_rcpf(ex[e] + 1.0f);
#pragma unroll
        for (int e = 0; e < 4; ++e) v[e] *= ex[e];
        u32x2_t o;
        o.x = pack_bf16x2(v[0], v[1]);
        o.y = pack_bf16x2(v[2], v[3]);
        return o;
    };
    auto load_ab = [&](const Blk& d, int c_lo, int n, float* fa, float* fb) __attribute__((always_inline)) {
        if (d.tab >= 0) {
            const f32x4_t* tp = (const f32x4_t*)(ldsTab + d.tab + chunk * 64 + c_lo * 8);
            for (int e = 0; e < n / 2; ++e) {
                const f32x4_t t = tp[e];
                fa[2 * e] = t.x; fb[2 * e] = t.y; fa[2 * e + 1] = t.z; fb[2 * e + 1] = t.w;
            }
        } else {
            for (int e = 0; e < n; ++e) { fa[e] = d.scale; fb[e] = 0.f; }
        }
    };
    auto zero_fill = [&](const Blk& d, unsigned st) __attribute__((always_inline)) {
        if (d.edge) {
            const u32x4_t z = u32x4_t{0u, 0u, 0u, 0u};
            if ((d.edge & 1) && srow == 0) *(u32x4_t*)(smem + st + wave * 1024 + lane_lds) = z;
            if ((d.edge & 2) && wave == 0 && lane >= 8 && lane < 16) *(u32x4_t*)(smem + st + HP * 1024 + lane_lds) = z;
        }
    };
    auto transform_all = [&](const Blk& d, unsigned st) __attribute__((always_inline)) {
        char* const ldsA = smem + st + wave * 1024 + lane_lds;
        if (d.tab < 0) {
            if (d.scale != 1.0f) {
                const float sc = d.scale;
#pragma unroll
                for (int u = 0; u < 2 * MH; ++u) {
                    const u32x4_t q = *(const u32x4_t*)(ldsA + u * 8192);
                    u32x4_t o;
                    o.x = pack_bf16x2(__uint_as_float(q.x << 16) * sc, __uint_as_float(q.x & 0xffff0000u) * sc);
                    o.y = pack_bf16x2(__uint_as_float(q.y << 16) * sc, __uint_as_float(q.y & 0xffff0000u) * sc);
                    o.z = pack_bf16x2(__uint_as_float(q.z << 16) * sc, __uint_as_float(q.z & 0xffff0000u) * sc);
                    o.w = pack_bf16x2(__uint_as_float(q.w << 16) * sc, __uint_as_float(q.w & 0xffff0000u) * sc);
                    *(u32x4_t*)(ldsA + u * 8192) = o;
                }
            }
            return;
        }
        char* const ldsH = smem + st + HP * 1024 + lane_lds;
        const bool halo = wave == 0 && d.taps == 3 && lane < 16;
        const bool act = true;
        float fa[8], fb[8];
        load_ab(d, 0, 8, fa, fb);
#pragma unroll
        for (int u = 0; u < 2 * MH; ++u) {
            const u32x4_t q = *(const u32x4_t*)(ldsA + u * 8192);
            const u32x2_t lo = silu4(u32x2_t{q.x, q.y}, fa, fb, act), hi = silu4(u32x2_t{q.z, q.w}, fa + 4, fb + 4, act);
            *(u32x4_t*)(ldsA + u * 8192) = u32x4_t{lo.x, lo.y, hi.x, hi.y};
        }
        if (halo) {
            const u32x4_t q = *(const u32x4_t*)ldsH;
            const u32x2_t lo = silu4(u32x2_t{q.x, q.y}, fa, fb, act), hi = silu4(u32x2_t{q.z, q.w}, fa + 4, fb + 4, act);
            *(u32x4_t*)ldsH = u32x4_t{lo.x, lo.y, hi.x, hi.y};
        }
        zero_fill(d, st);
    };

    f32x16_t acc[NH][MH][2];
    unsigned abase0[3];
#pragma unroll
    for (int t = 0; t < 3; ++t) {
        const int row = wm * 32 * MH + r + t, f = (row >> 1) & 7;
        abase0[t] = (unsigned)(row * kPpRow + ((h ^ (f & 1)) << 4) + ((f >> 1) << 5));
    }
    const int fw = (r >> 1) & 7;
    const unsigned wbase0 = (unsigned)((wn * 64 + r) * kPpRow + ((h ^ (fw & 1)) << 4) + ((fw >> 1) << 5));
    unsigned wadr[4];
#pragma unroll
    for (int ks = 0; ks < 4; ++ks) wadr[ks] = (unsigned)kPpOffW + (wbase0 ^ (unsigned)(ks << 5));

    unsigned ws0 = 0u, ws1 = (unsigned)kPpWStage, ws2 = 2u * (unsigned)kPpWStage;
    auto substep = [&](auto tapc, auto wstc, auto nhc, unsigned sa_, auto work, auto mid) __attribute__((always_inline)) {
        constexpr int TAP = decltype(tapc)::value;
        constexpr int WST = decltype(wstc)::value;
        constexpr int H = decltype(nhc)::value;
        const char* const pw = smem + (W3 ? ws0 : (unsigned)(WST * kPpWStage));
        unsigned aadr[4];
#pragma unroll
        for (int ks = 0; ks < 4; ++ks) aadr[ks] = sa_ + (abase0[TAP] ^ (unsigned)(ks << 5));
        bf16x8_t fa[2][MH], fb[2][2];
#pragma unroll
        for (int i = 0; i < MH; ++i) fa[0][i] = *(const bf16x8_t*)(smem + aadr[0] + i * 32 * kPpRow);
#pragma unroll
        for (int j = 0; j < 2; ++j) fb[0][j] = *(const bf16x8_t*)(pw + wadr[0] + j * 32 * kPpRow);
#pragma unroll
        for (int ks = 0; ks < 4; ++ks) {
            const int cur = ks & 1, nxt = cur ^ 1;
            if (ks + 1 < 4) {
#pragma unroll
                for (int i = 0; i < MH; ++i) fa[nxt][i] = *(const bf16x8_t*)(smem + aadr[ks + 1] + i * 32 * kPpRow);
#pragma unroll
                for (int j = 0; j < 2; ++j) fb[nxt][j] = *(const bf16x8_t*)(pw + wadr[ks + 1] + j * 32 * kPpRow);
            }
#pragma unroll
            for (int i = 0; i < MH; ++i)
#pragma unroll
                for (int j = 0; j < 2; ++j) {
                    if (!(ADF_RB_KNOCK & 8)) acc[H][i][j] = __builtin_amdgcn_mfma_f32_32x32x16_bf16(fa[cur][i], fb[cur][j], acc[H][i][j], 0, 0, 0);
                    else { asm volatile("" :: "v"(fa[cur][i]), "v"(fb[cur][j])); }
                    __builtin_amdgcn_sched_barrier(0);
                    if (!(ADF_RB_KNOCK & 1)) work(ks * 2 * MH + i * 2 + j);
                    __builtin_amdgcn_sched_barrier(0);
                }
            mid(ks);
            if (ADF_RB_PRIO == 4) {
                if (ks == 0) __builtin_amdgcn_s_setprio(2);
                else if (ks == 1) __builtin_amdgcn_s_setprio(1);
                else if (ks == 2) __builtin_amdgcn_s_setprio(0);
            }
            if (ADF_RB_PRIO == 2 && ks == 1 && wave >= 4) __builtin_amdgcn_s_setprio(2);
            if (ADF_RB_PRIO == 3 && ks == 1 && wave >= 4) __builtin_amdgcn_s_setprio(0);
            __builtin_amdgcn_sched_barrier(0);
        }
        if (ADF_RB_PRIO == 2 && wave >= 4) __builtin_amdgcn_s_setprio(0);
        if (ADF_RB_PRIO == 3 && wave >= 4) __builtin_amdgcn_s_setprio(2);
        if (ADF_RB_PRIO == 4) __builtin_amdgcn_s_setprio(3);
    };

    struct Part {
        u32x2_t raw[3];
        float ta[8], tb[8];
        float x[4], u[4];
        u32x2_t pk;
        float ec, ed;
        unsigned hraw;
        float ha, hb, hx, hu;
    };
    const unsigned halo_e = (unsigned)wave * 16u + ((unsigned)lane & 15u);
    auto half_of = [](int P, int k) constexpr -> int { return P < 2 ? P + 2 * k : 6 + k; };
    auto part_begin = [&](auto partc, const Blk& dn, unsigned sn, Part& p) __attribute__((always_inline)) {
        constexpr int P = decltype(partc)::value;
        char* const ldsN = smem + sn + wave * 1024 + lane_lds;
        if (P == 0) {
            load_ab(dn, 0, 4, p.ta, p.tb);
            p.ec = dn.tab >= 0 ? -1.4426950408889634f : 0.0f;
            p.ed = dn.tab >= 0 ? 0.0f : -200.0f;
        } else if (P == 1) load_ab(dn, 4, 4, p.ta + 4, p.tb + 4);
        constexpr int NOWN = MH == 2 ? (P < 2 ? 3 : 2) : (P < 2 ? 2 : 0);
#pragma unroll
        for (int k = 0; k < NOWN; ++k) {
            const int hh = half_of(P, k);
            p.raw[k] = *(const u32x2_t*)(ldsN + (hh >> 1) * 8192 + (hh & 1) * 8);
        }
        if (P == 2) {
            p.hraw = *(const unsigned short*)(smem + sn + HP * 1024 + halo_e * 2u);
            if (dn.tab >= 0) {
                const f32x2_t t = *(const f32x2_t*)(ldsTab + dn.tab + (halo_e & 63u) * 8u);
                p.ha = t.x; p.hb = t.y;
            } else { p.ha = dn.scale; p.hb = 0.f; }
        }
    };
    auto part_gap = [&](auto partc, const Blk& dn, unsigned sn, Part& p, int q) __attribute__((always_inline)) {
        constexpr int P = decltype(partc)::value;
        constexpr int NG = MH == 2 ? (P < 2 ? 3 : 2) : (P < 2 ? 2 : 0);
        constexpr int OPG = NG * 32 / (8 * MH * NH);
        char* const ldsN = smem + sn + wave * 1024 + lane_lds;
        if (P == 2 && q % NH == 0 && q / NH < 8) {
            switch (q / NH) {
                case 0: p.hx = __uint_as_float(p.hraw << 16); break;
                case 1: p.hx = fmaf(p.hx, p.ha, p.hb); break;
                case 2: p.hu = fmaf(p.hx, p.ec, p.ed); break;
                case 3: p.hu = __builtin_amdgcn_exp2f(p.hu); break;
                case 4: p.hu = p.hu + 1.0f; break;
                case 5: p.hu = __builtin_amdgcn_rcpf(p.hu); break;
                case 6: p.hx = p.hx * p.hu; break;
                default:
                    if (dn.taps == 3 && !((dn.edge & 2) && wave >= 4)) {
                        if (lane < 16) *(unsigned short*)(smem + sn + HP * 1024 + halo_e * 2u) = (unsigned short)pack_bf16x2(p.hx, p.hx);
                    }
                    break;
            }
        }
#pragma unroll
        for (int n = q * OPG; n < (q + 1) * OPG; ++n) {
            const int k = n >> 5, st = (n >> 2) & 7, j = n & 3;
            if (k >= NG) continue;
            const int hh = half_of(P, k);
            const int ch = (hh & 1) * 4 + j;
            switch (st) {
                case 0: {
                    const unsigned w = (j & 2) ? p.raw[k].y : p.raw[k].x;
                    p.x[j] = __uint_as_float((j & 1) ? (w & 0xffff0000u) : (w << 16));
                    break;
                }
                case 1: p.x[j] = fmaf(p.x[j], p.ta[ch], p.tb[ch]); break;
                case 2: p.u[j] = fmaf(p.x[j], p.ec, p.ed); break;
                case 3: p.u[j] = __builtin_amdgcn_exp2f(p.u[j]); break;
                case 4: p.u[j] = p.u[j] + 1.0f; break;
                case 5: p.u[j] = __builtin_amdgcn_rcpf(p.u[j]); break;
                case 6: p.x[j] = p.x[j] * p.u[j]; break;
                default:
                    if (j == 0) p.pk.x = pack_bf16x2(p.x[0], p.x[1]);
                    else if (j == 1) p.pk.y = pack_bf16x2(p.x[2], p.x[3]);
                    else if (j == 2) *(u32x2_t*)(ldsN + (hh >> 1) * 8192 + (hh & 1) * 8) = p.pk;
                    break;
            }
        }
#pragma unroll
        for (int j = 0; j < 4; ++j) { asm volatile("" : "+v"(p.x[j])); asm volatile("" : "+v"(p.u[j])); }
        if (P == 2) { asm volatile("" : "+v"(p.hx)); asm volatile("" : "+v"(p.hu)); }
    };
    auto part_end = [&](const Blk& dn, unsigned sn) __attribute__((always_inline)) { zero_fill(dn, sn); };

    const int cc = lane & 7, rsub = lane >> 3;
    auto epilogue = [&](const Tile& g, int next_n0, unsigned scr_stage) __attribute__((always_inline)) {
        float* const sc0 = (float*)(smem + scr_stage + wave * 4096);
        T* out = (T*)H.out;
        const bool stats_here = H.stats != nullptr;
        const int gs = stats_here ? (H.stats_mod ? H.stats_mod : H.n) / H.stats_groups : 8;
        const int tpg = gs / 8;
        const int mw0 = g.m0 + wm * 32 * MH;
        const T* resp = (const T*)H.res;
        const bool has_res = resp != nullptr;
        constexpr int PH = 4 * MH;
        constexpr int P = NH * PH;
        auto res_off = [&](int pass) __attribute__((always_inline)) -> unsigned {
            const int hf = pass / PH, q = pass % PH;
            const int m = mw0 + (q >> 2) * 32 + 8 * (q & 3) + rsub;
            return (unsigned)((g.b0 * H.L + m) * H.n + g.n0 + hf * kPpTN + wn * 64 + cc * 8);
        };
        float nb_[NH][2];
#pragma unroll
        for (int hf = 0; hf < NH; ++hf)
#pragma unroll
            for (int j = 0; j < 2; ++j) nb_[hf][j] = ldsBias[next_n0 + hf * kPpTN + wn * 64 + j * 32 + r];
        auto wr = [&](auto pc) __attribute__((always_inline)) {
            constexpr int p = decltype(pc)::value;
            constexpr int hf = p / PH, i = (p >> 2) % MH, p4 = p & 3;
            float* const scw = sc0 + (p & 1) * 512 + (4 * h) * 64 + r;
#pragma unroll
            for (int j = 0; j < 2; ++j)
#pragma unroll
                for (int e4 = 0; e4 < 4; ++e4) {
                    scw[e4 * 64 + j * 32] = acc[hf][i][j][4 * p4 + e4];
                    acc[hf][i][j][4 * p4 + e4] = nb_[hf][j];
                }
            __builtin_amdgcn_fence(__ATOMIC_RELEASE, "wavefront");
            __builtin_amdgcn_wave_barrier();
        };
        struct Row { float4 q0, q1; u32x4_t res; };
        auto rd = [&](auto pc, Row& rw) __attribute__((always_inline)) {
            constexpr int p = decltype(pc)::value;
            const float* const scr = sc0 + (p & 1) * 512 + rsub * 64 + cc * 8;
            rw.q0 = *(const float4*)(scr);
            rw.q1 = *(const float4*)(scr + 4);
            if (has_res) rw.res = (ADF_RB_NT & 2) ? __builtin_nontemporal_load((const u32x4_t*)(resp + res_off(p))) : *(const u32x4_t*)(resp + res_off(p));
            __builtin_amdgcn_fence(__ATOMIC_RELEASE, "wavefront");
            __builtin_amdgcn_wave_barrier();
        };
        f32x2_t s1v = {0.f, 0.f}, s2v = {0.f, 0.f};
        auto flush_stats = [&](int hf) __attribute__((always_inline)) {
            if (stats_here) {
                const int ncol = g.n0 + hf * kPpTN + wn * 64 + cc * 8;
                const int n = H.stats_mod ? (ncol & (H.stats_mod - 1)) : ncol;
                float s1 = s1v.x + s1v.y, s2 = s2v.x + s2v.y;
                for (int o = 1; o < tpg; o <<= 1) { s1 += __shfl_xor(s1, o, 64); s2 += __shfl_xor(s2, o, 64); }
                for (int o = 8; o < 64; o <<= 1) { s1 += __shfl_xor(s1, o, 64); s2 += __shfl_xor(s2, o, 64); }
                if (lane < 8 && (cc & (tpg - 1)) == 0) {
                    double* sp = H.stats + ((size_t)g.b0 * H.stats_groups + n / gs) * 2;
                    atomicAdd(sp, (double)s1);
                    atomicAdd(sp + 1, (double)s2);
                }
            }
            s1v = f32x2_t{0.f, 0.f}; s2v = f32x2_t{0.f, 0.f};
        };
        auto process = [&](auto pc, const Row& rw) __attribute__((always_inline)) {
            constexpr int p = decltype(pc)::value;
            float v[8];
            v[0] = rw.q0.x; v[1] = rw.q0.y; v[2] = rw.q0.z; v[3] = rw.q0.w; v[4] = rw.q1.x; v[5] = rw.q1.y; v[6] = rw.q1.z; v[7] = rw.q1.w;
            if (has_res) {
                float rf[8];
                unpack16<T>(rw.res, rf);
#pragma unroll
                for (int e = 0; e < 8; ++e) v[e] += rf[e];
            }
#if ADF_RB_DOT2
            const u32x4_t pk = pack16<T>(v);
            if (ADF_RB_NT & 1) __builtin_nontemporal_store(pk, (u32x4_t*)(out + res_off(p)));
            else *(u32x4_t*)(out + res_off(p)) = pk;
            {
                typedef __attribute__((ext_vector_type(2))) __bf16 bf2_t;
                const bf2_t one2 = __builtin_bit_cast(bf2_t, 0x3f803f80u);
                const unsigned w4[4] = {pk.x, pk.y, pk.z, pk.w};
#pragma unroll
                for (int e = 0; e < 4; ++e) {
                    const bf2_t q2 = __builtin_bit_cast(bf2_t, w4[e]);
                    if (e & 1) { s1v.y = __builtin_amdgcn_fdot2_f32_bf16(q2, one2, s1v.y, false); s2v.y = __builtin_amdgcn_fdot2_f32_bf16(q2, q2, s2v.y, false); }
                    else { s1v.x = __builtin_amdgcn_fdot2_f32_bf16(q2, one2, s1v.x, false); s2v.x = __builtin_amdgcn_fdot2_f32_bf16(q2, q2, s2v.x, false); }
                }
            }
#else
            if (ADF_RB_NT & 1) __builtin_nontemporal_store(pack16_stored<T>(v), (u32x4_t*)(out + res_off(p)));
            else *(u32x4_t*)(out + res_off(p)) = pack16_stored<T>(v);
#pragma unroll
            for (int e = 0; e < 8; e += 2) {
                const f32x2_t v2 = {v[e], v[e + 1]};
                s1v += v2;
                s2v += v2 * v2;
            }
#endif
            if (p % PH == PH - 1) flush_stats(p / PH);
        };
        Row rows[2];
        wr(std::integral_constant<int, 0>{});
        wr(std::integral_constant<int, 1>{});
        rd(std::integral_constant<int, 0>{}, rows[0]);
        rb_static_for<0, P>([&](auto pc) __attribute__((always_inline)) {
            constexpr int p = decltype(pc)::value;
            if (ADF_RB_PRIO == 4 && p > 0 && (p * 4) % P == 0) __builtin_amdgcn_s_setprio(3 - (p * 4) / P);
            if constexpr (p + 1 < P) rd(std::integral_constant<int, p + 1>{}, rows[(p + 1) & 1]);
            if constexpr (p + 2 < P) wr(std::integral_constant<int, p + 2>{});
            process(pc, rows[p & 1]);
        });
        if (ADF_RB_PRIO == 4) __builtin_amdgcn_s_setprio(3);
    };

#ifdef ADF_RB_STAMP
    auto kstamp = [&](int id) __attribute__((always_inline)) {
        if (bidx == 0) {
            const unsigned long long t = __builtin_amdgcn_s_memtime();
            if (lane == 0) ((unsigned long long*)(smem + kPpOffBias + 1024))[wave * 16 + id] = t;
        }
    };
#else
    auto kstamp = [&](int) __attribute__((always_inline)) {};
#endif
#ifdef ADF_RB_TL
    const int tl_which = bidx == 0 ? 0 : (bidx == (int)gridDim.x / 2 + 3 ? 1 : -1);
    unsigned* const tl_lds = (unsigned*)(smem + kPpOffBias + 1024) + wave * 128;
    auto tl = [&](int id) __attribute__((always_inline)) {
        if (tl_which >= 0 && id < 128) {
            const unsigned long long t = __builtin_amdgcn_s_memtime();
            if (lane == 0) tl_lds[id] = (unsigned)t;
        }
    };
    auto tl_real = [&](int id) __attribute__((always_inline)) {
        if (tl_which >= 0) {
            const unsigned long long t = __builtin_amdgcn_s_memrealtime();
            if (lane == 0) { tl_lds[id] = (unsigned)t; tl_lds[id + 1] = (unsigned)(t >> 32); }
        }
    };
    if (tl_which >= 0) for (int i = lane; i < 128; i += 64) tl_lds[i] = 0u;
    int tl_sub = 0;
    tl_real(120);
    tl(0);
#else
    auto tl = [&](int) __attribute__((always_inline)) {};
#endif
    kstamp(11);
    tl(110);
    const bool hb0 = H.bias0 != nullptr, hb1 = H.bias1 != nullptr;
    const float* const dummy_f = (const float*)a.blk[0].w;
    const int bidx_l = tid < H.n ? tid : 0;
    const float b0v = (hb0 ? H.bias0 : dummy_f)[bidx_l], b1v = (hb1 ? H.bias1 : dummy_f)[bidx_l];
    GnLoaded gl = {};
    if constexpr (!RAW) gl = gn_load(b_first, tid < ctot0 ? tid : ctot0 - 1);
    tl(111);
    Blk dc = make_desc_of(e_first[0]);
    advance();
    issue_a01(dc, 0u); issue_a23(dc, 0u); issue_halo(dc, 0u);
    issue_w(dc.w, 0);
    if (W3 && !ADF_RB_FILL2) issue_w(dc.w + (unsigned)(1 / NH) * slab + (unsigned)(1 % NH) * (unsigned)kPpWStage, 1);
    Blk d1 = make_desc_of(e_first[1]);
    advance();
    if (!ADF_RB_FILL2) { issue_a01(d1, (unsigned)kPpAStage); issue_a23(d1, (unsigned)kPpAStage); issue_halo(d1, (unsigned)kPpAStage); }
    Blk d2 = make_desc_of(d_k == 0 ? e_first[0] : e_first[2]);
    advance();
    tl(112);
#ifdef ADF_RB_TL
    asm volatile("" :: "v"(gl.gamma), "v"(gl.beta), "v"(gl.f1s), "v"(gl.f1h), "v"(gl.f2s), "v"(gl.f2h), "v"(gl.s0), "v"(gl.q0), "v"(gl.s1), "v"(gl.q1), "v"(b0v), "v"(b1v));
    tl(113);
#endif
    if (tid < H.n) ldsBias[tid] = (hb0 ? b0v : 0.f) + (hb1 ? b1v : 0.f);
    if (!RAW && tid < ctot0) gn_store(tid, gl, 0);
    kstamp(12);
    tl(1);
    asm volatile("s_waitcnt vmcnt(0)" ::: "memory");
    if (ADF_RB_FILL2) {
        if (W3) issue_w(dc.w + (unsigned)(1 / NH) * slab + (unsigned)(1 % NH) * (unsigned)kPpWStage, 1);
        issue_a01(d1, (unsigned)kPpAStage); issue_a23(d1, (unsigned)kPpAStage); issue_halo(d1, (unsigned)kPpAStage);
    }
    __syncthreads();
    kstamp(13);
    tl(2);
    Tile cur_tile = tile_of(0);
#pragma unroll
    for (int hf = 0; hf < NH; ++hf) {
        float bias_r[2];
#pragma unroll
        for (int j = 0; j < 2; ++j) bias_r[j] = ldsBias[cur_tile.n0 + hf * kPpTN + wn * 64 + j * 32 + r];
#pragma unroll
        for (int i = 0; i < MH; ++i)
#pragma unroll
            for (int j = 0; j < 2; ++j)
#pragma unroll
                for (int e = 0; e < 16; ++e) acc[hf][i][j][e] = bias_r[j];
    }
    if (RAW) zero_fill(dc, 0u); else transform_all(dc, 0u);
    if (ADF_RB_FILL2) asm volatile("s_waitcnt vmcnt(0)" ::: "memory");
    asm volatile("s_waitcnt lgkmcnt(0)\n\ts_barrier" ::: "memory");
    kstamp(14);
    tl(3);

    unsigned sa = 0u, sa1 = (unsigned)kPpAStage, sa2 = 2u * (unsigned)kPpAStage;
    const std::integral_constant<int, 0> c0{};
    const std::integral_constant<int, 1> c1{};
    const std::integral_constant<int, 2> c2{};
    auto lds_barrier = [&]() __attribute__((always_inline)) { asm volatile("s_waitcnt lgkmcnt(0)\n\ts_barrier" ::: "memory"); };
    auto rotate = [&]() __attribute__((always_inline)) {
        const unsigned t = sa; sa = sa1; sa1 = sa2; sa2 = t;
        dc = d1; d1 = d2; d2 = make_desc();
        advance();
    };
    int tseq = 0, kb = 0;
    bool prev_one = false;
    int remaining = ntiles * nb;

    auto next_slab = [&](int u, int taps_) __attribute__((always_inline)) -> const char* {
        return dc.w + (unsigned)(u / NH) * slab + (unsigned)(u % NH) * (unsigned)kPpWStage;
    };
    auto slab_of = [&](const Blk& d, int v) __attribute__((always_inline)) -> const char* {
        return d.w + (unsigned)(v / NH) * slab + (unsigned)(v % NH) * (unsigned)kPpWStage;
    };
    auto issue_ahead = [&](int v, int ucur, bool has1, bool has2) __attribute__((always_inline)) -> int {
        if (v < ucur) { issue_w_at(slab_of(dc, v), ws2); return 2; }
        v -= ucur;
        if (!has1) return 0;
        const int u1 = d1.taps * NH;
        if (v < u1) { issue_w_at(slab_of(d1, v), ws2); return 2; }
        if (!has2) return 0;
        issue_w_at(slab_of(d2, v - u1), ws2);
        return 2;
    };
    auto wait_n = [&](int n) __attribute__((always_inline)) {
        if (n == 2) asm volatile("s_waitcnt vmcnt(2)" ::: "memory");
        else if (n == 4) asm volatile("s_waitcnt vmcnt(4)" ::: "memory");
        else if (n == 5) asm volatile("s_waitcnt vmcnt(5)" ::: "memory");
        else if (n >= 7) asm volatile("s_waitcnt vmcnt(7)" ::: "memory");
        else if (n == 6) asm volatile("s_waitcnt vmcnt(6)" ::: "memory");
        else if (n == 3) asm volatile("s_waitcnt vmcnt(3)" ::: "memory");
        else asm volatile("s_waitcnt vmcnt(0)" ::: "memory");
    };
    auto w_rotate = [&]() __attribute__((always_inline)) { const unsigned t = ws0; ws0 = ws1; ws1 = ws2; ws2 = t; };
    auto wait_upto = [&](int n) __attribute__((always_inline)) {
#define ADF_RB_WCASE(k) case k: asm volatile("s_waitcnt vmcnt(" #k ")" ::: "memory"); break;
        switch (n < 0 ? 0 : (n > 31 ? 31 : n)) {
            ADF_RB_WCASE(0) ADF_RB_WCASE(1) ADF_RB_WCASE(2) ADF_RB_WCASE(3) ADF_RB_WCASE(4) ADF_RB_WCASE(5) ADF_RB_WCASE(6) ADF_RB_WCASE(7)
            ADF_RB_WCASE(8) ADF_RB_WCASE(9) ADF_RB_WCASE(10) ADF_RB_WCASE(11) ADF_RB_WCASE(12) ADF_RB_WCASE(13) ADF_RB_WCASE(14) ADF_RB_WCASE(15)
            ADF_RB_WCASE(16) ADF_RB_WCASE(17) ADF_RB_WCASE(18) ADF_RB_WCASE(19) ADF_RB_WCASE(20) ADF_RB_WCASE(21) ADF_RB_WCASE(22) ADF_RB_WCASE(23)
            ADF_RB_WCASE(24) ADF_RB_WCASE(25) ADF_RB_WCASE(26) ADF_RB_WCASE(27) ADF_RB_WCASE(28) ADF_RB_WCASE(29) ADF_RB_WCASE(30)
            default: asm volatile("s_waitcnt vmcnt(31)" ::: "memory"); break;
        }
#undef ADF_RB_WCASE
    };
    int epi_vm = 0;
    bool slab1_pre = false;
    int aq_prev = 0;
    auto block3 = [&](auto wpc) __attribute__((always_inline)) {
        constexpr int WP = decltype(wpc)::value;
        constexpr int U = 3 * NH;
#ifdef ADF_RB_STAMP
        const bool stamp_on = bidx == 0 && tseq == 1 && kb == 2 && WP == 0;
        auto stamp = [&](int id) __attribute__((always_inline)) {
            if (stamp_on && id < 16) {
                const unsigned long long t = __builtin_amdgcn_s_memtime();
                if (lane == 0) ((unsigned long long*)(smem + kPpOffBias + 1024))[wave * 16 + id] = t;
            }
        };
#else
        auto stamp = [&](int) __attribute__((always_inline)) {};
#endif
        const bool has1 = remaining > 1, has2 = remaining > 2;
        if (prev_one) { asm volatile("s_waitcnt vmcnt(0)" ::: "memory"); aq_prev = 0; }
        Part part;
        stamp(0);
        rb_static_for<0, U>([&](auto uc) __attribute__((always_inline)) {
            constexpr int u = decltype(uc)::value;
            constexpr int TAP = u / NH, HF = u % NH;
            const std::integral_constant<int, TAP> tapc{};
            const std::integral_constant<int, (WP + u) & 1> wstc{};
            const std::integral_constant<int, HF> hfc{};
            if (HF == 0 && !RAW) part_begin(tapc, d1, sa1, part);
            int wq = 0, aq = 0;
            substep(tapc, wstc, hfc, sa, [&](int q) __attribute__((always_inline)) { if (!RAW) part_gap(tapc, d1, sa1, part, HF * 8 * MH + q); },
                    [&](int ks) __attribute__((always_inline)) {
                        if (ks == 0) {
                            if (W3) wq = issue_ahead(u + 2, U, has1, has2);
                            else if (u + 1 < U) { if (!(u == 0 && slab1_pre)) issue_w(next_slab(u + 1, 3), (WP + u + 1) & 1); }
                            else if (has1) issue_w(d1.w, (WP + u + 1) & 1);
                        } else if (ks == 1 && has2) {
                            if (u == 0) { issue_halo(d2, sa2); issue_a01(d2, sa2); aq = (wave == 0 && d2.taps == 3) ? 3 : 2; }
                            else if (u == 1 && MH == 2) { issue_a23(d2, sa2); aq = 2; }
                        }
                    });
            if (u == U - 1) part_end(d1, sa1);
            stamp(3 * u + 1);
#ifdef ADF_RB_TL
            tl(4 + tseq * 26 + 2 + 2 * tl_sub);
#endif
            if (u == 0 && epi_vm > 0) {
                wait_upto(epi_vm + (W3 ? aq_prev + wq + aq : aq));
                epi_vm = 0; slab1_pre = false;
                if (W3) { aq_prev = aq; w_rotate(); }
            } else if (W3) {
                wait_n((u == U - 1 ? 0 : aq_prev) + wq + aq);
                aq_prev = aq;
                w_rotate();
            } else if ((u == 0 || (MH == 2 && u == 1)) && has2) asm volatile("s_waitcnt vmcnt(2)" ::: "memory");
            else asm volatile("s_waitcnt vmcnt(0)" ::: "memory");
            stamp(3 * u + 2);
            if (!RAW && u == 2 && kb == 0 && tseq + 1 < ntiles) {
                const Tile nt = tile_of(tseq + 1);
                if (nt.b0 != cur_tile.b0) fill_table(nt.b0, (nt.b0 - b_first) & 1);
            }
            lds_barrier();
            stamp(3 * u + 3);
#ifdef ADF_RB_TL
            tl(4 + tseq * 26 + 3 + 2 * tl_sub);
            ++tl_sub;
#endif
        });
#ifdef ADF_RB_STAMP
        if (stamp_on && lane < 16) adf_rb_stamps[wave * 16 + lane] = ((const unsigned long long*)(smem + kPpOffBias + 1024))[wave * 16 + lane];
#endif
    };
    auto block1 = [&](auto wpc) __attribute__((always_inline)) {
        constexpr int WP = decltype(wpc)::value;
        const bool has1 = remaining > 1, has2 = remaining > 2;
        rb_static_for<0, NH>([&](auto uc) __attribute__((always_inline)) {
            constexpr int u = decltype(uc)::value;
            const std::integral_constant<int, (WP + u) & 1> wstc{};
            const std::integral_constant<int, u> hfc{};
            int wq = 0, aq = 0;
            substep(c0, wstc, hfc, sa, [](int) __attribute__((always_inline)) {},
                    [&](int ks) __attribute__((always_inline)) {
                        if (ks == 0) {
                            if (W3) wq = issue_ahead(u + 2, NH, has1, has2);
                            else if (u + 1 < NH) issue_w(next_slab(u + 1, 1), (WP + u + 1) & 1);
                            else if (has1) issue_w(d1.w, (WP + u + 1) & 1);
                        } else if (u == NH - 1 && has2) {
                            if (ks == 1) { issue_a01(d2, sa2); aq += 2; }
                            else if (ks == 2) { issue_a23(d2, sa2); if (MH == 2) aq += 2; }
                            else { issue_halo(d2, sa2); if (wave == 0 && d2.taps == 3) aq += 1; }
                        }
                    });
            if (W3) {
                wait_n((u == NH - 1 ? 0 : aq_prev) + wq + aq);
                aq_prev = aq;
                w_rotate();
                if (u == NH - 1 && has1) transform_all(d1, sa1);
            } else if (u == NH - 1) {
                if (has2) {
                    if (MH == 2) { if (wave == 0 && d2.taps == 3) asm volatile("s_waitcnt vmcnt(5)" ::: "memory"); else asm volatile("s_waitcnt vmcnt(4)" ::: "memory"); }
                    else { if (wave == 0 && d2.taps == 3) asm volatile("s_waitcnt vmcnt(3)" ::: "memory"); else asm volatile("s_waitcnt vmcnt(2)" ::: "memory"); }
                }
                else asm volatile("s_waitcnt vmcnt(0)" ::: "memory");
                if (has1) transform_all(d1, sa1);
            } else {
                asm volatile("s_waitcnt vmcnt(0)" ::: "memory");
            }
            lds_barrier();
        });
    };
    constexpr int kPar3 = (3 * NH) & 1, kPar1 = NH & 1;

    for (; tseq < ntiles; ++tseq) {
        cur_tile = tile_of(tseq);
#ifdef ADF_RB_TL
        tl_sub = 0;
        tl(4 + tseq * 26);
#endif
        if (tseq > 0) {
#ifdef ADF_RB_STAMP
            if (tseq == 1) kstamp(15);
#endif
            if (ADF_RB_PRESLAB) {
                if (prev_one) { asm volatile("s_waitcnt vmcnt(0)" ::: "memory"); aq_prev = 0; prev_one = false; }
                if (!W3) { issue_w(next_slab(1, 3), 1); slab1_pre = true; }
                epi_vm = NH * 4 * MH * (H.res != nullptr ? 2 : 1) + (H.stats != nullptr ? 2 * NH : 0);
            }
            epilogue(tile_of(tseq - 1), cur_tile.n0, sa2);
        }
#ifdef ADF_RB_TL
        tl(4 + tseq * 26 + 1);
#endif
        for (kb = 0; kb < nb3; kb += 2) {
            block3(c0); rotate(); --remaining; prev_one = false;
            block3(std::integral_constant<int, kPar3>{}); rotate(); --remaining;
        }
        for (int k1 = 0; k1 < nb1; k1 += 2) {
            block1(c0); rotate(); --remaining;
            block1(std::integral_constant<int, kPar1>{}); rotate(); --remaining; prev_one = true;
        }
    }
    {
        const Tile last = tile_of(ntiles - 1);
        tl(108);
        epilogue(last, 0, sa2);
        tl(109);
    }
#ifdef ADF_RB_TL
    tl_real(122);
    if (tl_which >= 0) {
        asm volatile("s_waitcnt lgkmcnt(0)" ::: "memory");
        for (int i = lane; i < 128; i += 64) adf_rb_tl[(tl_which * 8 + wave) * 128 + i] = tl_lds[i];
    }
#endif
}

}
```

### audiodiffuser_amd/csrc/adf_net_unet1d.hip

```cpp
#include "adf_api_internal.h"

using namespace adf;
using namespace adf_api;

namespace adf_api {

struct ResW {
    int cin = 0, cout = 0, film_off = 0;
    float *g1w = nullptr, *g1b = nullptr, *g2w = nullptr, *g2b = nullptr;
    ConvW c1, c2, cr;
    bool has_res = false;
};
struct TrW {
    int c = 0, mid = 0;
    float *lnw = nullptr, *lnb = nullptr, *g0 = nullptr, *g3 = nullptr;
    ConvW qkv, proj, ff1, ff2;
};
struct DownW { ConvW down; std::vector<ResW> blocks; bool attn = false; TrW tr; int factor = 1, cin = 0, cout = 0; };
struct UpW { std::vector<ResW> blocks; bool attn = false; TrW tr; ConvW up; ConvW up3; int factor = 1, cin = 0, cout = 0; bool nearest = false; };

struct Unet1dNet : Net {
    adf_net_config cfg;
    float *to_in_w = nullptr, *to_out_w = nullptr, *fourier = nullptr, *t_w1 = nullptr, *t_b1 = nullptr, *t_w2 = nullptr, *t_b2 = nullptr;
    std::vector<DownW> downs;
// ... 101 lines not shown
    GemmArgs gemm_base(const Act& out, int lin, int mrows, const ConvW& w) {
        GemmArgs g;
        memset(&g, 0, sizeof(g));
        g.nseg = 1; g.B = p->B; g.lin = lin; g.mrows = mrows; g.n = w.n; g.n_pad = w.n_pad;
        g.bias0 = w.bias; g.bias_mod = w.n > 0 ? w.n : 1;
        g.out = out.p; g.out_rows = out.L; g.out_c = out.C;
        return g;
    }
    static GemmSeg seg_of(const Act& x, const Act* skip, const float* ab, float scale1, int act, int taps, int stride, int off0,
                          int step, const ConvW& w) {
        GemmSeg sg;
        memset(&sg, 0, sizeof(sg));
        sg.src0 = x.p; sg.c0 = x.C;
        sg.src1 = skip ? skip->p : nullptr; sg.c1 = skip ? skip->C : 0;
        sg.ab = ab; sg.scale1 = scale1; sg.act = act;
        sg.taps = taps; sg.stride = stride; sg.off0 = off0; sg.step = step;
        sg.w = w.w; sg.wfrag = w.wfrag; sg.nchunk = w.nchunk;
        return sg;
    }
    void run_gemm(GemmArgs& g, Act& out, bool want_stats) {
        const bool ask = want_stats && can_fuse_stats(out.C);
        if (ask) {
            out.stats = alloc_stats();
            g.stats = out.stats; g.stats_groups = c.resnet_groups;
        }
        if (live()) {
            bool fused = false;
            check(launch_conv_gemm(g, h->gemm_dtype(), s, &fused));
            if (ask && !fused) check(launch_gn_stats(out.p, h->bf16, p->B, out.L, out.C, c.resnet_groups, out.stats, s));
        }
    }

    Act linear(const Act& x, const ConvW& w, const void* res, int gelu, bool want_stats) {
        Act out = new_act(w.n, x.L);
        const int rows = p->B * x.L;
        GemmArgs g = gemm_base(out, rows, rows, w);
        g.B = 1; g.out_rows = rows;
        g.seg[0] = seg_of(x, nullptr, nullptr, 1.f, 0, 1, 1, 0, 1, w);
        g.res = res; g.gelu = gelu;
        run_gemm(g, out, false);
        (void)want_stats;
        return out;
    }

    Act resblock(const std::string& name, Act& x, Act* skip, const ResW& r, int nb) {
        const int B = p->B, G = c.resnet_groups;
        const float sscale = c.use_skip_scale ? 0.70710678118654752440f : 1.0f;
        const int ctot = x.C + (skip ? skip->C : 0);
        if (ctot != r.cin) check("resblock: channel mismatch");
        double* s0 = ensure_stats(x);
        double* s1 = skip ? ensure_stats(*skip) : nullptr;
        static int short_max = -1;
        if (short_max < 0) short_max = (int)adf_tuning("ADF_SHORT_LEVEL", 32);
        const bool short_level = x.L <= short_max && (x.L & (x.L - 1)) == 0;
        float* ab1 = (float*)alloc((size_t)B * ctot * 2 * 4);
        GnFinalizeArgs f1;
        memset(&f1, 0, sizeof(f1));
        f1.stats0 = s0; f1.stats1 = s1; f1.c0 = x.C; f1.c1 = skip ? skip->C : 0; f1.L = x.L; f1.G = G; f1.B = B;
        f1.scale1 = sscale; f1.eps = 1e-5f; f1.gamma = r.g1w; f1.beta = r.g1b; f1.film = nullptr; f1.ab = ab1;
        static int rb_fused = -1;
        if (rb_fused < 0) rb_fused = adf_route_switch("ADF_RB_FUSED", 2);
        if (rb_fused && h->bf16 && (x.L == 16 || x.L == 64) && r.cout == 256 && x.C == 256 && (!skip || skip->C == 256) && G == 8 &&
            r.c1.wfrag && r.c2.wfrag && (!r.has_res || r.cr.wfrag) && r.c1.n_pad == 256 && !(c.flags & ADF_FLAG_SEPARATE_GN_STATS)) {
            Act y = new_act(r.cout, x.L);
            RbFusedArgs fa;
            memset(&fa, 0, sizeof(fa));
            fa.x = (const bf16_t*)x.p; fa.skip = skip ? (const bf16_t*)skip->p : nullptr; fa.out = (bf16_t*)y.p;
            fa.gn1 = f1;
            fa.gamma2 = r.g2w; fa.beta2 = r.g2b;
            fa.film = film + r.film_off; fa.film_bstride = nb == 1 ? 0 : h->film_total;
            if (film2) { fa.film2 = film2 + r.film_off; fa.film2_bstride = film2_bstride; }
            fa.w1 = r.c1.wfrag; fa.w2 = r.c2.wfrag; fa.wr = r.has_res ? r.cr.wfrag : nullptr;
            fa.b1 = r.c1.bias; fa.b2 = r.c2.bias; fa.br = r.has_res ? r.cr.bias : nullptr;
            fa.skip_scale = sscale; fa.eps = 1e-5f;
            y.stats = alloc_stats(); fa.stats = y.stats;
            if (rb_fused >= 2 && B * 4 <= 256) {
                Act hact = new_act(r.cout, x.L);
                RbSplitArgs sa;
                sa.f = fa; sa.hact = (bf16_t*)hact.p;
                if (live()) check(launch_resblock_split(sa, B, x.L, ctot, s));
            } else if (live()) check(launch_resblock_small(fa, B, x.L, ctot, s));
            RbRec rec{name, GemmArgs{}, GemmArgs{}, r.cin, r.cout, x.L};
            rec.g1.nseg = 0;
            p->rbs.push_back(rec);
            tap(name, y);
            return y;
        }
        Act h1 = new_act(r.cout, x.L);
        GemmArgs g1 = gemm_base(h1, x.L, x.L, r.c1);
        if (short_level) {
            Act a1 = new_act(ctot, x.L);
            if (live()) check(launch_gn_norm_apply(x.p, skip ? skip->p : nullptr, f1, 1, a1.p, h->bf16, s));
            g1.seg[0] = seg_of(a1, nullptr, nullptr, 1.f, 0, 3, 1, -1, 1, r.c1);
        } else {
            g1.seg[0] = seg_of(x, skip, ab1, sscale, 1, 3, 1, -1, 1, r.c1);
            g1.seg[0].gn = f1;
        }
        run_gemm(g1, h1, true);
        tap(name + ".h1", h1);
        double* sh = ensure_stats(h1);
        float* ab2 = (float*)alloc((size_t)B * r.cout * 2 * 4);
        GnFinalizeArgs f2;
        memset(&f2, 0, sizeof(f2));
        f2.stats0 = sh; f2.c0 = r.cout; f2.L = x.L; f2.G = G; f2.B = B; f2.scale1 = 1.f; f2.eps = 1e-5f;
        f2.gamma = r.g2w; f2.beta = r.g2b;
        f2.film = film + r.film_off; f2.film_bstride = nb == 1 ? 0 : h->film_total; f2.ab = ab2;
        if (film2) { f2.film2 = film2 + r.film_off; f2.film2_bstride = film2_bstride; }
        Act y = new_act(r.cout, x.L);
        GemmArgs g2 = gemm_base(y, x.L, x.L, r.c2);
        if (short_level) {
            Act a2 = new_act(r.cout, x.L);
            if (live()) check(launch_gn_norm_apply(h1.p, nullptr, f2, 1, a2.p, h->bf16, s));
            g2.seg[0] = seg_of(a2, nullptr, nullptr, 1.f, 0, 3, 1, -1, 1, r.c2);
        } else {
            g2.seg[0] = seg_of(h1, nullptr, ab2, 1.f, 1, 3, 1, -1, 1, r.c2);
            g2.seg[0].gn = f2;
        }
        if (r.has_res) {
            g2.nseg = 2;
            g2.seg[1] = seg_of(x, skip, nullptr, sscale, 0, 1, 1, 0, 1, r.cr);
            g2.bias1 = r.cr.bias;
        } else {
            if (skip) check("resblock: identity residual with a skip input");
            g2.res = x.p;
        }
        run_gemm(g2, y, true);
        p->rbs.push_back({name, g1, g2, r.cin, r.cout, x.L});
        tap(name, y);
        return y;
    }

    Act transformer(const std::string& name, Act& x, const TrW& t) {
        const long long rows = (long long)p->B * x.L;
        static int tr_fused = -1;
        if (tr_fused < 0) tr_fused = adf_route_switch("ADF_TR_FUSED", 2);
        if (tr_fused && h->bf16 && t.c == 256 && t.mid == 512 && c.attention_heads == 8 && (x.L == 16 || x.L == 64) &&
            x.C == 256 && t.qkv.nchunk == 4 && t.ff2.nchunk == 8 && t.qkv.wfrag) {
            Act x2 = new_act(t.c, x.L);
            TrFusedArgs fa;
            memset(&fa, 0, sizeof(fa));
            fa.x = (const bf16_t*)x.p; fa.out = (bf16_t*)x2.p;
            fa.ln_w = t.lnw; fa.ln_b = t.lnb; fa.g0 = t.g0; fa.g3 = t.g3;
            fa.wqkv = t.qkv.wfrag; fa.wproj = t.proj.wfrag; fa.wff1 = t.ff1.wfrag; fa.wff2 = t.ff2.wfrag;
            fa.npad_qkv = t.qkv.n_pad; fa.npad_proj = t.proj.n_pad; fa.npad_ff1 = t.ff1.n_pad; fa.npad_ff2 = t.ff2.n_pad;
            fa.eps = 1e-5f;
            if (c.resnet_groups == 8 && !(c.flags & ADF_FLAG_SEPARATE_GN_STATS)) { x2.stats = alloc_stats(); fa.stats = x2.stats; }
            if (live()) check(launch_transformer_small(fa, p->B, x.L, s));
            tap(name, x2);
            return x2;
        }
        if (tr_fused >= 2 && h->bf16 && t.c == 256 && t.mid == 512 && c.attention_heads == 8 && x.L % 64 == 0 && x.L > 64 &&
            x.C == 256 && t.qkv.nchunk == 4 && t.ff2.nchunk == 8 && t.qkv.wfrag && c.resnet_groups == 8 &&
            !(c.flags & ADF_FLAG_SEPARATE_GN_STATS)) {
            Act qkv = new_act(3 * t.c, x.L), att = new_act(t.c, x.L), x2 = new_act(t.c, x.L);
            TrFusedArgs fa;
            memset(&fa, 0, sizeof(fa));
            fa.x = (const bf16_t*)x.p; fa.out = (bf16_t*)x2.p; fa.qkv_out = (bf16_t*)qkv.p; fa.att = (const bf16_t*)att.p;
            fa.ln_w = t.lnw; fa.ln_b = t.lnb; fa.g0 = t.g0; fa.g3 = t.g3;
            fa.wqkv = t.qkv.wfrag; fa.wproj = t.proj.wfrag; fa.wff1 = t.ff1.wfrag; fa.wff2 = t.ff2.wfrag;
            fa.npad_qkv = t.qkv.n_pad; fa.npad_proj = t.proj.n_pad; fa.npad_ff1 = t.ff1.n_pad; fa.npad_ff2 = t.ff2.n_pad;
            fa.eps = 1e-5f;
            x2.stats = alloc_stats(); fa.stats = x2.stats;
            if (live()) {
                check(launch_transformer_tiles(fa, (int)rows, x.L, 1, s));
                check(launch_attention(qkv.p, att.p, h->bf16, p->B, x.L, t.c, c.attention_heads, s));
                check(launch_transformer_tiles(fa, (int)rows, x.L, 2, s));
            }
            tap(name + ".qkv", qkv);
            tap(name + ".att", att);
            tap(name, x2);
            return x2;
        }
        Act xn = new_act(t.c, x.L);
        if (live()) check(launch_ln_rows(x.p, xn.p, h->bf16, rows, t.c, t.lnw, t.lnb, 1e-5f, s));
        tap(name + ".ln", xn);
        Act qkv = linear(xn, t.qkv, nullptr, 0, false);
        tap(name + ".qkv", qkv);
        Act att = new_act(t.c, x.L);
        if (live()) check(h->x3 ? launch_attention_x3(qkv.p, att.p, p->B, x.L, t.c, c.attention_heads, s)
                                : launch_attention(qkv.p, att.p, h->bf16, p->B, x.L, t.c, c.attention_heads, s));
        tap(name + ".att", att);
        Act x1 = linear(att, t.proj, x.p, 0, false);
        tap(name + ".x1", x1);
        Act n1 = new_act(t.c, x.L);
        if (live()) check(launch_ln_rows(x1.p, n1.p, h->bf16, rows, t.c, t.g0, nullptr, 1e-5f, s));
        tap(name + ".n1", n1);
        Act f1 = linear(n1, t.ff1, nullptr, 1, false);
        tap(name + ".f1", f1);
        Act n2 = new_act(t.mid, x.L);
        if (live()) check(launch_ln_rows(f1.p, n2.p, h->bf16, rows, t.mid, t.g3, nullptr, 1e-5f, s));
        tap(name + ".n2", n2);
        Act x2 = linear(n2, t.ff2, x1.p, 0, true);
        tap(name, x2);
        return x2;
    }
};

int Unet1dNet::build_weights(adf_handle* h) {
    const adf_net_config& c = cfg;
    Registrar1d R{{h}};
    const int ch = c.channels, tdim = 4 * ch, n = c.num_layers;
    if (c.num_classes > 0) R.label_embedder(ch, tdim, c.num_classes);
    const int temb = tdim + h->cdim;
    to_in_w = R.reg_f32("unet.to_in.to_in.weight", (int64_t)c.num_filters * c.in_channels * c.window_length);
    to_out_w = R.reg_f32("unet.to_out.to_out.weight", (int64_t)c.num_filters * c.out_channels * c.window_length);
    fourier = R.reg_f32("unet.to_time.0.0.weights", ch / 2);
    t_w1 = R.reg_f32("unet.to_time.0.1.weight", (int64_t)tdim * (ch + 1));
    t_b1 = R.reg_f32("unet.to_time.0.1.bias", tdim);
    t_w2 = R.reg_f32("unet.to_time.2.weight", (int64_t)tdim * tdim);
    t_b2 = R.reg_f32("unet.to_time.2.bias", tdim);
    downs.resize(n);
    for (int i = 0; i < n; ++i) {
        DownW& d = downs[i];
        d.cin = ch * c.multipliers[i]; d.cout = ch * c.multipliers[i + 1]; d.factor = c.factors[i];
        const std::string pre = "unet.downsamples." + std::to_string(i);
        R.conv_folded(pre + ".downsample", d.down, d.cout, d.cin, d.factor * c.kernel_multiplier_downsample + 1, d.factor);
        d.blocks.resize(c.num_blocks[i]);
        for (int j = 0; j < c.num_blocks[i]; ++j) R.resblock(pre + ".blocks." + std::to_string(j), d.blocks[j], d.cout, d.cout, temb);
        d.attn = c.attentions[i] != 0;
        if (d.attn) R.transformer(pre + ".transformer", d.tr, d.cout, c.attention_multiplier);
    }
    const int cb = ch * c.multipliers[n];
    R.resblock("unet.bottleneck.pre_block", mid_pre, cb, cb, temb);
    if (c.use_attention_bottleneck) R.transformer("unet.bottleneck.transformer", mid_tr, cb, c.attention_multiplier);
    R.resblock("unet.bottleneck.post_block", mid_post, cb, cb, temb);
    ups.resize(n);
    for (int u = 0; u < n; ++u) {
        const int i = n - 1 - u;
        UpW& up = ups[u];
        up.cin = ch * c.multipliers[i + 1]; up.cout = ch * c.multipliers[i]; up.factor = c.factors[i];
        const std::string pre = "unet.upsamples." + std::to_string(u);
        const int nb = c.num_blocks[i] + (c.attentions[i] ? 1 : 0);
        up.blocks.resize(nb);
        for (int j = 0; j < nb; ++j) R.resblock(pre + ".blocks." + std::to_string(j), up.blocks[j], 2 * up.cin, up.cin, temb);
        up.attn = c.attentions[i] != 0;
        if (up.attn) R.transformer(pre + ".transformer", up.tr, up.cin, c.attention_multiplier);
        const int f = up.factor;
        if (c.flags & ADF_FLAG_NEAREST_UPSAMPLE) {
            up.nearest = true;
            R.conv(pre + ".upsample.2", up.up, up.cout, up.cin, 3, true);
            continue;
        }
        R.reg_pack(pre + ".upsample.weight", up.up, up.cout, up.cin, 2 * f, 0, f * up.cout, true, f);
        if (h->bf16 && up.up.w && (up.cin == 128 || up.cin == 256) && (up.cout == 64 || up.cout == 128 || up.cout == 256) && (f == 2 || f == 4)) {
            up.up.wfrag = dalloc(h, (size_t)up.up.nchunk * up.up.taps * up.up.n_pad * kRowBytes);
            if (!up.up.wfrag) R.ok = false;
            else h->slots[pre + ".upsample.weight"].frag = up.up.wfrag;
        }
        up.up.bias = R.reg_f32(pre + ".upsample.bias", up.cout);
        if ((h->bf16 || h->x3) && up.up.w && f == 2 && (f * up.cout == 128 || f * up.cout == 256) && up.cin % 128 == 0 && up.cout % 64 == 0) {
            ConvW& w3 = up.up3;
            w3.cin = up.cin; w3.K = 2 * f; w3.f = f; w3.taps = 3;
            w3.n = f * up.cout; w3.n_pad = w3.n; w3.cout = w3.n;
            w3.nchunk = ceil_div(up.cin, h->kc);
            w3.w = dalloc(h, ((size_t)w3.nchunk * 3 * w3.n_pad + (size_t)kTapGroup * (w3.n_pad + 128)) * kRowBytes);
            w3.bias = (float*)dalloc(h, (size_t)w3.n * 4);
            if (!w3.w || !w3.bias) R.ok = false;
            else {
                Slot& sw = h->slots[pre + ".upsample.weight"];
                sw.dst3 = w3.w; sw.n_pad3 = w3.n_pad;
                Slot& sb = h->slots[pre + ".upsample.bias"];
                sb.rep = w3.bias; sb.rep_n = f;
            }
        }
    }
    h->film_w = (float*)dalloc(h, (size_t)h->film_total * temb * 4);
    h->film_b = (float*)dalloc(h, (size_t)h->film_total * 4);
    if (!h->film_w || !h->film_b) R.ok = false;
    for (const auto& fn : R.film_names) {
        R.reg_f32(fn.pre + ".to_cond_embedding.1.weight", (int64_t)fn.rows * temb, h->film_w + (size_t)fn.off * temb);
        R.reg_f32(fn.pre + ".to_cond_embedding.1.bias", fn.rows, h->film_b + fn.off);
    }
    return R.ok ? 0 : fail(h, "device allocation failed while building the weight registry");
}

int Unet1dNet::forward(adf_handle* h, Plan* p, const FwdIO& io, hipStream_t s) {
    const adf_net_config& c = cfg;
    Walker1d W{{h, p, s}, c};
    W.film2 = io.film2; W.film2_bstride = io.film2_bstride;
    W.film = io.film_pre ? io.film_pre : p->film;
    if (W.begin()) return 1;
    const int B = p->B, L = p->L, n = c.num_layers;
    const int pad = c.window_length / 2 - c.stride / 2;
    const int tdim = 4 * c.channels;
    if (W.live() && !io.film_pre) {
        W.check(time_embed(io.t, io.t_stride, io.nb, p->temb, s));
        W.check(launch_film(p->temb, tdim, h->film_w, tdim + h->cdim, 0, h->film_b, p->film, io.nb, h->film_total, s));
    }
    Act x = W.new_act(c.num_filters, L / c.stride);
    if (W.live())
        W.check(launch_to_in(io.x, to_in_w, x.p, h->bf16, B, c.in_channels, L, c.num_filters, c.window_length, c.stride, pad,
                             io.coef, io.coef_bstride, s));
    W.tap("to_in", x);
    std::vector<std::vector<Act>> skips_list;
    for (int i = 0; i < n; ++i) {
        const DownW& d = downs[i];
        const int f = d.factor, km = c.kernel_multiplier_downsample;
        Act y = W.new_act(d.cout, x.L / f);
        if (x.L % f) return fail(h, "downsample: length not divisible by the factor");
        Act xv = x;
        xv.C = x.C * f; xv.L = x.L / f; xv.stats = nullptr;
        GemmArgs g = W.gemm_base(y, xv.L, y.L, d.down);
        g.seg[0] = Walker1d::seg_of(xv, nullptr, nullptr, 1.f, 0, km + 1, 1, -(km / 2), 1, d.down);
        W.run_gemm(g, y, true);
        W.tap("down" + std::to_string(i) + ".conv", y);
        x = y;
        std::vector<Act> skips;
        for (size_t j = 0; j < d.blocks.size(); ++j) {
            x = W.resblock("down" + std::to_string(i) + ".block" + std::to_string(j), x, nullptr, d.blocks[j], io.nb);
            skips.push_back(x);
        }
        if (d.attn) {
            x = W.transformer("down" + std::to_string(i) + ".attn", x, d.tr);
            skips.push_back(x);
        }
        skips_list.push_back(skips);
    }
    x = W.resblock("mid.pre", x, nullptr, mid_pre, io.nb);
    if (c.use_attention_bottleneck) x = W.transformer("mid.attn", x, mid_tr);
    x = W.resblock("mid.post", x, nullptr, mid_post, io.nb);
    for (int u = 0; u < n; ++u) {
        const UpW& up = ups[u];
        std::vector<Act>& skips = skips_list.back();
        for (size_t j = 0; j < up.blocks.size(); ++j) {
            if (skips.empty()) { W.check("upsample: skip stack underflow"); break; }
            Act sk = skips.back();
            skips.pop_back();
            x = W.resblock("up" + std::to_string(u) + ".block" + std::to_string(j), x, &sk, up.blocks[j], io.nb);
        }
        skips_list.pop_back();
        if (up.attn) x = W.transformer("up" + std::to_string(u) + ".attn", x, up.tr);
        const int f = up.factor;
        Act y = W.new_act(up.cout, x.L * f);
        bool done = false;
        if (up.nearest) {
            Act u0 = W.new_act(up.cin, x.L * f + 2);
            if (W.live()) W.check(launch_upsample_nearest_pad(x.p, u0.p, h->bf16, B, x.L, up.cin, f, s));
            GemmArgs g = W.gemm_base(y, x.L * f + 2, x.L * f, up.up);
            g.seg[0] = Walker1d::seg_of(u0, nullptr, nullptr, 1.f, 0, 3, 1, 0, 1, up.up);
            W.run_gemm(g, y, u + 1 < n);
            done = true;
        }
        if (up.up3.w) {
            Act y3 = y;
            y3.C = f * up.cout; y3.L = x.L;
            GemmArgs g3 = W.gemm_base(y3, x.L, x.L, up.up3);
            g3.seg[0] = Walker1d::seg_of(x, nullptr, nullptr, 1.f, 0, 3, 1, -1, 1, up.up3);
            g3.phase_c = up.cout;
            if (conv_gemm_phase_eligible(g3, h->gemm_dtype())) {
                W.run_gemm(g3, y, u + 1 < n);
                done = true;
            }
        }
        if (!done) {
            GemmArgs g = W.gemm_base(y, x.L, x.L + 1, up.up);
            g.seg[0] = Walker1d::seg_of(x, nullptr, nullptr, 1.f, 0, 2, 1, 0, -1, up.up);
            g.bias_mod = up.cout;
            g.scatter_f = f; g.scatter_pad = f / 2 + f % 2;
            W.run_gemm(g, y, u + 1 < n);
        }
        W.tap("up" + std::to_string(u) + ".conv", y);
        x = y;
    }
    if (W.live())
        W.check(launch_to_out(x.p, to_out_w, io.out, h->gemm_dtype(), B, c.out_channels, x.L, c.num_filters, c.window_length, c.stride, pad,
                              io.mode, io.x_noisy, io.coef, io.coef_bstride, s));
    return W.bad ? 1 : 0;
}

}

extern "C" int adf_create(const adf_net_config* cfg, adf_handle** out) {
    if (create_begin("adf_create", cfg, out)) return 1;
    const adf_net_config& c = *cfg;
    if (c.num_layers < 1 || c.num_layers > ADF_MAX_LAYERS) { g_create_error = "adf_create: bad num_layers"; return 1; }
    if (c.num_filters != c.channels * c.multipliers[0]) { g_create_error = "adf_create: num_filters must equal channels*multipliers[0]"; return 1; }
    if (c.channels % 2 || c.channels < 2) { g_create_error = "adf_create: channels must be even"; return 1; }
    if (c.dtype != ADF_DTYPE_F32 && c.dtype != ADF_DTYPE_BF16 && c.dtype != ADF_DTYPE_F32X3) { g_create_error = "adf_create: bad dtype"; return 1; }
    auto net = std::make_unique<Unet1dNet>();
    net->cfg = c;
    NetDims& d = net->dims;
    d.in_channels = c.in_channels; d.out_channels = c.out_channels;
    d.length_multiple = c.stride;
    for (int i = 0; i < c.num_layers; ++i) d.length_multiple *= c.factors[i];
    d.temb = 4 * c.channels; d.label_in = c.channels; d.num_classes = c.num_classes; d.stat_groups = c.resnet_groups;
    return create_finish("adf_create", c.dtype, std::move(net), out);
}
```

### include/audiodiffuser_amd.h

```cpp
#ifndef AUDIODIFFUSER_AMD_H
#define AUDIODIFFUSER_AMD_H

#include <stdint.h>

#ifdef __cplusplus
extern "C" {
#endif

#define ADF_ABI_VERSION 7
int adf_abi_version(void);

#define ADF_MAX_LAYERS 12

#define ADF_DTYPE_F32 0
#define ADF_DTYPE_BF16 1
#define ADF_DTYPE_F32X3 2

typedef struct adf_net_config {
    int32_t channels, num_filters, window_length, stride, in_channels, out_channels;
    int32_t resnet_groups, kernel_multiplier_downsample;
    int32_t num_layers;
    int32_t multipliers[ADF_MAX_LAYERS + 1];
    int32_t factors[ADF_MAX_LAYERS];
    int32_t num_blocks[ADF_MAX_LAYERS];
    int32_t attentions[ADF_MAX_LAYERS];
    int32_t attention_heads, attention_multiplier;
    int32_t use_skip_scale, use_attention_bottleneck;
    int32_t dtype;
    int32_t flags;
    int32_t num_classes;
} adf_net_config;

#define ADF_FLAG_SEPARATE_GN_STATS 1
#define ADF_FLAG_NEAREST_UPSAMPLE 2

#define ADF_SAMPLER_EDM 0
#define ADF_SAMPLER_EDM_ALPHA 1
#define ADF_SAMPLER_DPM_MULTISTEP 2
#define ADF_SAMPLER_DPM2 3
#define ADF_SAMPLER_ADPM2 4
#define ADF_SAMPLER_LMS 5
#define ADF_SAMPLER_DPM2M 7
#define ADF_SAMPLER_UNIPC 8
#define ADF_SAMPLER_DPM_SINGLESTEP 6
#define ADF_SAMPLER_ADPMPP2S 9
#define ADF_SAMPLER_RF_EULER 10

typedef struct adf_sampler_desc {
    int32_t kind;
    int32_t num_steps;
    float s_tmin, s_tmax, s_churn, s_noise;
    int32_t use_heun;
    float alpha;
    int32_t order;
    float sigma_data;
    int32_t use_graph;
    float rho, eta;
    int32_t log_time_spacing;
    int32_t eps_pred;
    int32_t reflow;
} adf_sampler_desc;

typedef struct adf_wavenet_config {
    int32_t residual_channels, residual_layers, dilation_cycle;
    int32_t dim_in, dim_mid, dim_out;
    int32_t dtype;
} adf_wavenet_config;

#define ADF_ADM_MAX_LEVELS 8
typedef struct adf_adm_config {
    int32_t in_channels, model_channels, out_channels, num_res_blocks;
    int32_t n_mult; int32_t channel_mult[ADF_ADM_MAX_LEVELS];
    int32_t n_attention_ds; int32_t attention_ds[ADF_ADM_MAX_LEVELS];
    int32_t conv_resample, num_heads, num_head_channels, use_scale_shift_norm, resblock_updown, use_new_attention_order;
    int32_t num_classes;
    int32_t dtype;
} adf_adm_config;

#define ADF_U2D_MAX_LEVELS 8
#define ADF_U2D_MAX_INIT_KERNELS 4
typedef struct adf_unet2d_config {
    double ff_mult;
    int32_t dim, cond_dim, channels, channels_out, num_classes;
    int32_t n_levels; int32_t dim_mults[ADF_U2D_MAX_LEVELS];
    int32_t layer_attns[ADF_U2D_MAX_LEVELS]; int32_t layer_cross_attns[ADF_U2D_MAX_LEVELS];
    int32_t num_resnet_blocks, resnet_groups, attn_heads;
    int32_t layer_attns_depth, layer_mid_attns_depth, attend_at_middle;
    int32_t n_init_kernels; int32_t init_kernel_sizes[ADF_U2D_MAX_INIT_KERNELS];
    int32_t learned_sinu_pos_emb_dim, num_time_tokens;
    int32_t scale_skip_connection, final_resnet_block;
    int32_t dtype;
} adf_unet2d_config;

typedef struct adf_handle adf_handle;

int adf_create(const adf_net_config* cfg, adf_handle** out);
int adf_adm_create(const adf_adm_config* cfg, adf_handle** out);
int adf_unet2d_create(const adf_unet2d_config* cfg, adf_handle** out);
int adf_set_image_shape(adf_handle* h, int H, int W);

int adf_set_dynamic_threshold(adf_handle* h, float quantile);

#define ADF_PRECOND_EDM 0
#define ADF_PRECOND_VE 1
#define ADF_PRECOND_VP 2
#define ADF_PRECOND_V_EDM 3
#define ADF_PRECOND_RF 4
#define ADF_PRECOND_RF_EDM 5
int adf_set_preconditioning(adf_handle* h, int kind, double beta_min, double beta_d, double M);
int adf_wavenet_create(const adf_wavenet_config* cfg, adf_handle** out);
void adf_destroy(adf_handle* h);
const char* adf_last_error(const adf_handle* h);

int adf_num_weights(const adf_handle* h);
const char* adf_weight_name(const adf_handle* h, int index);
int64_t adf_weight_numel(const adf_handle* h, int index);
int adf_load_weight(adf_handle* h, const char* name, const float* dev_fp32, int64_t numel, void* stream);
int adf_weights_missing(const adf_handle* h);

int adf_set_condition(adf_handle* h, const int64_t* classes_dev, int B, int null_labels, float cond_scale, void* stream);

int adf_net_forward(adf_handle* h, const float* x, const float* t, float* out, int B, int L, void* stream);

int adf_denoise(adf_handle* h, const float* x_noisy, const float* sigmas_dev, float sigma, float sigma_data,
                float* out, int B, int L, void* stream);

#define ADF_LOSS_X0_EDM        0
#define ADF_LOSS_X0_INV_SIGMA2 1
#define ADF_LOSS_RF            2
int adf_diffusion_loss(adf_handle* h, int kind, const float* x, const float* noise, const float* sigmas_dev, float sigma_data,
                       float* losses, float* x_noisy_out, float* pred_out, int B, int L, void* stream);
int64_t adf_loss_calls(const adf_handle* h);

int adf_sampler_run(adf_handle* h, const adf_sampler_desc* desc, const float* sigmas_host, int n_sigmas,
                    const float* noise, const float* injected_noise, int n_injected, float* out, int B, int L, void* stream);
int adf_sampler_nfe(const adf_sampler_desc* desc, const float* sigmas_host, int n_sigmas);

int adf_debug_tap_shape(adf_handle* h, const char* name, int* C, int* L);
int adf_debug_tap_copy(adf_handle* h, const char* name, float* out_fp32, void* stream);
int adf_debug_tap_stats(adf_handle* h, const char* name, double* out_host, int* groups, void* stream);
int adf_debug_up_tile_plan(int cin, int cout, int f, int B, int L, int* tile_rows, int* items, int* rounds, int* dead_rows);
int adf_debug_dyn_threshold(adf_handle* h, float* x_dev, int B, long long per_sample, float quantile, void* stream);
int adf_debug_coef_rows(adf_handle* h, float* out_dev, int max_rows, int* n_rows, void* stream);
int adf_debug_tap_count(adf_handle* h);
const char* adf_debug_tap_name(adf_handle* h, int index);

typedef struct adf_run_counters {
    int64_t sampler_runs;
    int64_t sampler_evals;
    int64_t graph_captures;
    int64_t graph_replays;
    int64_t denoise_calls;
    int64_t net_passes;
} adf_run_counters;
int adf_get_counters(const adf_handle* h, adf_run_counters* out);

int64_t adf_device_bytes(const adf_handle* h);

int adf_bench_resblock(adf_handle* h, int B, int L, int level, int iters, float* ms_block1, float* ms_block2,
                       double* algo_bytes_block1, double* algo_bytes_block2, double* flops_block1,
                       double* flops_block2, void* stream);
int adf_bench_layer(adf_handle* h, int B, int L, int level, int conv, int iters, float* ms, double* algo_bytes, double* flops,
                    int* copies, void* stream);

int adf_bench_wavenet_layer(adf_handle* h, int B, int T, int layer, int iters, float* ms, double* algo_bytes, double* flops, void* stream);

int adf_bench_loss_kernels(adf_handle* h, int rf, int B, long long N, int iters, float* ms_mix, float* ms_partial, double* bytes_mix,
                           double* bytes_partial, void* stream);

typedef struct adf_istft_config {
    int32_t n_fft, hop_length, center, normalized;
    double spec_abs_exponent, spec_factor;
} adf_istft_config;
typedef struct adf_istft_plan adf_istft_plan;
int adf_istft_create(const adf_istft_config* cfg, const float* window, adf_istft_plan** out);
int adf_istft_basis(const adf_istft_config* cfg, const float* window, float* basis, float* wsq);
int adf_istft_run(adf_istft_plan* plan, const float* spec, int B, int T, float* audio, int64_t audio_len, void* stream);
void adf_istft_destroy(adf_istft_plan* plan);

typedef struct adf_stft_plan adf_stft_plan;
int adf_stft_create(const adf_istft_config* cfg, const float* window, adf_stft_plan** out);
int adf_stft_basis(const adf_istft_config* cfg, const float* window, float* basis);
int adf_stft_run(adf_stft_plan* plan, const float* audio, int B, int64_t L, float* spec, int T, void* stream);
void adf_stft_destroy(adf_stft_plan* plan);

#ifdef __cplusplus
}
#endif
#endif
```

Baseline: 4.467 million audio-samples/s.

## Skip structurally zero third-tap weights in folded downsample conv GEMM

For a strided downsample conv that has been folded into a three-tap GEMM over f*C channels, the third tap's weights are zero for the trailing channel blocks. The host now computes where that zero region starts and tells the rb kernel to run those K-blocks as two-tap blocks instead of three-tap, skipping MFMA work and weight loads. It also adds a phase-split variant for the phase_c path, where each N half needs only two taps, plus a debug entry point that reports the block plan. This adds template variants and more complex pipeline scheduling, with a risk of wait-count and pipeline mismatches in the new two-tap blocks.

```diff
diff --git a/audiodiffuser_amd/_lib.py b/audiodiffuser_amd/_lib.py
--- a/audiodiffuser_amd/_lib.py
+++ b/audiodiffuser_amd/_lib.py
@@ -128,6 +128,7 @@
     "adf_debug_tap_shape": (C.c_int, [C.c_void_p, C.c_char_p, C.POINTER(C.c_int), C.POINTER(C.c_int)]),
     "adf_debug_tap_copy": (C.c_int, [C.c_void_p, C.c_char_p, C.c_void_p, C.c_void_p]),
     "adf_debug_tap_stats": (C.c_int, [C.c_void_p, C.c_char_p, C.c_void_p, C.POINTER(C.c_int), C.c_void_p]),
+    "adf_debug_rb_block_plan": (C.c_int, [C.c_int] * 9 + [C.POINTER(C.c_int)] * 5),
     "adf_debug_up_tile_plan": (C.c_int, [C.c_int, C.c_int, C.c_int, C.c_int, C.c_int, C.POINTER(C.c_int), C.POINTER(C.c_int), C.POINTER(C.c_int),
                                          C.POINTER(C.c_int)]),
     "adf_debug_dyn_threshold": (C.c_int, [C.c_void_p, C.c_void_p, C.c_int, C.c_longlong, C.c_float, C.c_void_p]),
diff --git a/audiodiffuser_amd/csrc/adf_gemm.h b/audiodiffuser_amd/csrc/adf_gemm.h
--- a/audiodiffuser_amd/csrc/adf_gemm.h
+++ b/audiodiffuser_amd/csrc/adf_gemm.h
@@ -18,7 +18,16 @@
     const void* w;
     const void* wfrag;
     int nchunk;
+    int tap2_zero_c;
 };
+
+inline int folded_tap2_zero_from(int K, int f, int C) {
+    if (f < 1 || C < 1 || (K - 1) / f + 1 != 3) return 0;
+    int z = f;
+    for (int j = f - 1; j >= 0 && 2 * f + j >= K; --j) z = j;
+    if (z == 0 || z == f || f + (f - 1) >= K) return 0;
+    return (z * C) % 64 == 0 ? z * C : 0;
+}
 
 struct GemmArgs {
     GemmSeg seg[2];
diff --git a/audiodiffuser_amd/csrc/adf_gemm.hip b/audiodiffuser_amd/csrc/adf_gemm.hip
--- a/audiodiffuser_amd/csrc/adf_gemm.hip
+++ b/audiodiffuser_amd/csrc/adf_gemm.hip
@@ -173,7 +173,7 @@
 }
 
 template <typename ArgsT>
-void rb_fill_args(const GemmArgs& a, const RbForm& f, const RbTiles& t, ArgsT& r) {
+void rb_fill_args(const GemmArgs& a, const RbForm& f, const RbTiles& t, int zskip, ArgsT& r) {
     const GemmSeg& g0 = a.seg[0];
     memset(&r, 0, sizeof(r));
     int nb = 0;
@@ -193,6 +193,14 @@
     if (a.nseg > 1) add_seg(a.seg[1].src0, a.seg[1].src1, a.seg[1].c0, a.seg[1].c1, a.seg[1].w, 1, false, a.seg[1].scale1);
     r.h.res = a.nseg == 1 ? a.res : nullptr;
     r.h.nb1 = nb - r.h.nb3;
+    if (zskip && rb_raw0(a)) {
+        const int z = g0.tap2_zero_c, nbz = z / f.blk_ch;
+        if (!a.phase_c && z > 0 && z % f.blk_ch == 0 && nbz >= 2 && nbz % 2 == 0 && nbz < r.h.nb3) {
+            r.h.nb2 = r.h.nb3 - nbz;
+            r.h.nb3 = nbz;
+        }
+        if (a.phase_c && a.n == 2 * a.phase_c && t.nh == 2) r.h.phase2 = 1;
+    }
     r.h.B = a.B; r.h.L = a.mrows;
     r.h.n = a.n;
     r.h.gn = g0.gn;
@@ -207,18 +215,24 @@
     r.h.tiles_total = (int)t.total;
 }
 
-const char* launch_rb(const GemmArgs& a, long long min_tiles, hipStream_t stream) {
+const char* launch_rb(const GemmArgs& a, long long min_tiles, int zskip, hipStream_t stream) {
     RbTiles t;
     RbArgs r;
     rb_tiles(a, kRbBf16, min_tiles, t);
-    rb_fill_args(a, kRbBf16, t, r);
+    rb_fill_args(a, kRbBf16, t, zskip, r);
+    if (r.h.nb2 && (r.h.nb3 < 2 || r.h.nb3 % 2 || r.h.nb1)) return "conv_gemm_rb: two-tap blocks need an even number >= 2 of three-tap blocks ahead of them";
     if (!raise_lds_limit<kRbLds, conv_gemm_rb_kernel<1, false, 2>, conv_gemm_rb_kernel<2, false, 2>, conv_gemm_rb_kernel<1, true, 2>, conv_gemm_rb_kernel<2, true, 2>,
                          conv_gemm_rb_kernel<1, false, 1>, conv_gemm_rb_kernel<2, false, 1>, conv_gemm_rb_kernel<1, true, 1>, conv_gemm_rb_kernel<2, true, 1>>())
         return "hipFuncSetAttribute(MaxDynamicSharedMemorySize, rb) failed";
     const long long grid = t.total < device_cus() ? t.total : device_cus();
     const bool raw0 = rb_raw0(a);
     auto go = [&](auto kern) { hipLaunchKernelGGL(kern, dim3((unsigned)grid), dim3(512), kRbLds, stream, r); };
-    if (t.tm == 256) {
+    if (r.h.phase2) {
+        if (!raise_lds_limit<kRbLds, conv_gemm_rb_kernel<2, true, 2, true>, conv_gemm_rb_kernel<2, true, 1, true>>())
+            return "hipFuncSetAttribute(MaxDynamicSharedMemorySize, rb) failed";
+        if (t.tm == 256) go(conv_gemm_rb_kernel<2, true, 2, true>);
+        else go(conv_gemm_rb_kernel<2, true, 1, true>);
+    } else if (t.tm == 256) {
         if (t.nh == 2 && raw0) go(conv_gemm_rb_kernel<2, true, 2>);
         else if (t.nh == 2) go(conv_gemm_rb_kernel<2, false, 2>);
         else if (raw0) go(conv_gemm_rb_kernel<1, true, 2>);
@@ -236,7 +250,7 @@
     RbTiles t;
     Rbx3Args r;
     rb_tiles(a, kRbX3, min_tiles, t);
-    rb_fill_args(a, kRbX3, t, r);
+    rb_fill_args(a, kRbX3, t, 0, r);
     if (!raise_lds_limit<kRbLds, conv_gemm_rbx3_kernel<2>, conv_gemm_rbx3_kernel<1>>()) return "hipFuncSetAttribute(MaxDynamicSharedMemorySize, rbx3) failed";
     const long long grid = t.total < device_cus() ? t.total : device_cus();
     if (t.tm == 256) hipLaunchKernelGGL(conv_gemm_rbx3_kernel<2>, dim3((unsigned)grid), dim3(512), kRbLds, stream, r);
@@ -312,6 +326,7 @@
     int ws = adf_route_switch("ADF_GEMM_WS", 1);
     long long rb_min_tiles = min_tiles_of(adf_route_switch("ADF_GEMM_RB", 1));
     long long rbx3_min_tiles = min_tiles_of(adf_route_switch("ADF_GEMM_RBX3", 1));
+    int rb_zskip = adf_route_switch("ADF_RB_ZSKIP", 1);
     int gn_in_kernel = (int)adf_tuning("ADF_GEMM_GN", 1);
     int min_blocks = (int)adf_tuning("ADF_GEMM_MINBLOCKS", 512);
     int ksplit = (int)adf_tuning("ADF_GEMM_KSPLIT", 1);
@@ -544,7 +559,7 @@
         if (p.tm == 64) return dtype == 1 ? launch_ksplit<bf16_t, 2, 2>(a, stream) : (dtype == 2 ? launch_ksplit<f32x3_t, 2, 2>(a, stream) : launch_ksplit<float, 2, 2>(a, stream));
         return dtype == 1 ? launch_ksplit<bf16_t, 1, 1>(a, stream) : (dtype == 2 ? launch_ksplit<f32x3_t, 1, 1>(a, stream) : launch_ksplit<float, 1, 1>(a, stream));
     case Route::rbx3: return launch_rbx3(a, sw.rbx3_min_tiles, stream);
-    case Route::rb: return launch_rb(a, sw.rb_min_tiles, stream);
+    case Route::rb: return launch_rb(a, sw.rb_min_tiles, sw.rb_zskip, stream);
     case Route::pp: return p.tm == 256 ? launch_pp<2>(a, stream) : launch_pp<1>(a, stream);
     case Route::ws:
         if (p.tn == 128) return dtype == 1 ? launch_ws_variant<bf16_t, 2, 2>(a, stream) : launch_ws_variant<float, 2, 2>(a, stream);
@@ -553,6 +568,32 @@
     }
 }
 
+}
+
+extern "C" int adf_debug_rb_block_plan(int K, int f, int C, int phase_c, int n, int B, int L, int min_tiles, int zskip, int* tile_rows, int* nh, int* nb3, int* nb2,
+                                       int* phase2) {
+    using namespace adf;
+    if (B < 1 || L < 1 || C < 1 || f < 1 || (long long)B * L > 0x3fffffffLL) return 1;
+    static const char dummy[16] = {};
+    GemmArgs a;
+    memset(&a, 0, sizeof(a));
+    a.nseg = 1; a.B = B; a.lin = a.mrows = a.out_rows = L; a.n = a.n_pad = a.out_c = a.bias_mod = n;
+    a.phase_c = phase_c;
+    GemmSeg& g = a.seg[0];
+    g.src0 = g.w = dummy;
+    g.c0 = phase_c ? C : f * C;
+    g.taps = 3; g.stride = 1; g.off0 = -1; g.step = 1;
+    g.tap2_zero_c = phase_c ? 0 : folded_tap2_zero_from(K, f, C);
+    RbTiles t;
+    if (!rb_shape_ok(a, kRbBf16, false) || !rb_tiles(a, kRbBf16, min_tiles, t)) return 1;
+    RbArgs r;
+    rb_fill_args(a, kRbBf16, t, zskip, r);
+    if (tile_rows) *tile_rows = t.tm;
+    if (nh) *nh = t.nh;
+    if (nb3) *nb3 = r.h.nb3;
+    if (nb2) *nb2 = r.h.nb2;
+    if (phase2) *phase2 = r.h.phase2;
+    return 0;
 }
 
 extern "C" int adf_debug_up_tile_plan(int cin, int cout, int f, int B, int L, int* tile_rows, int* items, int* rounds, int* dead_rows) {
diff --git a/audiodiffuser_amd/csrc/adf_gemm_rb.h b/audiodiffuser_amd/csrc/adf_gemm_rb.h
--- a/audiodiffuser_amd/csrc/adf_gemm_rb.h
+++ b/audiodiffuser_amd/csrc/adf_gemm_rb.h
@@ -61,6 +61,8 @@
     const void* res;
     double* stats; int stats_groups;
     int stats_mod;
+    int nb2;
+    int phase2;
 };
 struct RbArgs {
     RbHead h;
@@ -84,8 +86,9 @@
     }
 }
 
-template <int NH, bool RAW, int MH = 2>
+template <int NH, bool RAW, int MH = 2, bool PHASE = false>
 __global__ void __launch_bounds__(512) conv_gemm_rb_kernel(const RbArgs a) {
+    static_assert(!PHASE || (RAW && NH == 2), "the phase form: no prologue, N half = phase");
     typedef bf16_t T;
     constexpr int TM = 128 * MH, HP = TM / 8;
     constexpr int TNB = kPpTN * NH;
@@ -116,7 +119,8 @@
     const int t_hi = (int)((unsigned)(bidx + 1) * (unsigned)H.tiles_total / (unsigned)nblk_grid);
     const int ntiles = t_hi - t_lo;
     if (ntiles <= 0) return;
-    const int nb3 = H.nb3, nb1 = H.nb1, nb = nb3 + nb1;
+    const int nb3 = H.nb3, nb2 = RAW ? H.nb2 : 0, nb1 = H.nb1, nbh = nb3 + nb2, nb = nbh + nb1;
+    constexpr bool phase2 = PHASE;
     const int ctot0 = H.gn.c0 + H.gn.c1;
     const int tn_shift = H.tiles_n > 1 ? 1 : 0;
     const int tm_mask = (1 << H.tm_shift) - 1;
@@ -146,14 +150,14 @@
     Tile d_tile = tile_of(0);
     auto make_desc_of = [&](const RbBlk& e) __attribute__((always_inline)) -> Blk {
         Blk d;
-        const int three = d_k < nb3;
+        const int three = d_k < nbh;
         const int p_lo = d_tile.m0 - three;
         d.pitch = e.pitch;
         d.abase = e.src + (long long)(d_tile.b0 * H.L + p_lo) * (long long)e.pitch;
         d.w = e.w + (unsigned)d_tile.n0 * (unsigned)kRowBytes;
         d.tab = e.tab >= 0 ? ((d_tile.b0 - b_first) & 1) * kPpTab + e.tab : -1;
         d.scale = e.scale;
-        d.taps = three ? 3 : 1;
+        d.taps = three ? ((d_k < nb3 && !phase2) ? 3 : 2) : 1;
         d.edge = three ? ((d_tile.m0 == 0 ? 1 : 0) | (d_tile.m0 + TM >= H.L ? 2 : 0)) : 0;
         return d;
     };
@@ -165,6 +169,10 @@
         }
     };
     const unsigned slab = (unsigned)H.n * (unsigned)kRowBytes;
+    auto slab_of = [&](const Blk& d, int v) __attribute__((always_inline)) -> const char* {
+        const int tap = phase2 ? (v + 1) >> 1 : v / NH, hf = phase2 ? v >> 1 : v % NH;
+        return d.w + (unsigned)tap * slab + (unsigned)hf * (unsigned)kPpWStage;
+    };
 
     const unsigned colbytes = (unsigned)chunk * 16u;
     auto issue_a01 = [&](const Blk& d, unsigned st) __attribute__((always_inline)) {
@@ -182,7 +190,7 @@
     };
     auto issue_halo = [&](const Blk& d, unsigned st) __attribute__((always_inline)) {
         if (ADF_RB_KNOCK & 2) return;
-        if (wave == 0 && d.taps == 3) {
+        if (wave == 0 && d.taps > 1) {
             const unsigned vh = (unsigned)TM * d.pitch + ((d.edge & 2) ? 0u : (unsigned)lrow * d.pitch) + colbytes;
             if (lane < 16) rb_dma1(d.abase, vh, st + (unsigned)HP * 1024u);
         }
@@ -305,7 +313,7 @@
             return;
         }
         char* const ldsH = smem + st + HP * 1024 + lane_lds;
-        const bool halo = wave == 0 && d.taps == 3 && lane < 16;
+        const bool halo = wave == 0 && d.taps > 1 && lane < 16;
         const bool act = true;
         float fa[8], fb[8];
         load_ab(d, 0, 8, fa, fb);
@@ -432,7 +440,7 @@
                 case 5: p.hu = __builtin_amdgcn_rcpf(p.hu); break;
                 case 6: p.hx = p.hx * p.hu; break;
                 default:
-                    if (dn.taps == 3 && !((dn.edge & 2) && wave >= 4)) {
+                    if (dn.taps > 1 && !((dn.edge & 2) && wave >= 4)) {
                         if (lane < 16) *(unsigned short*)(smem + sn + HP * 1024 + halo_e * 2u) = (unsigned short)pack_bf16x2(p.hx, p.hx);
                     }
                     break;
@@ -627,7 +635,7 @@
     advance();
     issue_a01(dc, 0u); issue_a23(dc, 0u); issue_halo(dc, 0u);
     issue_w(dc.w, 0);
-    if (W3 && !ADF_RB_FILL2) issue_w(dc.w + (unsigned)(1 / NH) * slab + (unsigned)(1 % NH) * (unsigned)kPpWStage, 1);
+    if (W3 && !ADF_RB_FILL2) issue_w(slab_of(dc, 1), 1);
     Blk d1 = make_desc_of(e_first[1]);
     advance();
     if (!ADF_RB_FILL2) { issue_a01(d1, (unsigned)kPpAStage); issue_a23(d1, (unsigned)kPpAStage); issue_halo(d1, (unsigned)kPpAStage); }
@@ -644,7 +652,7 @@
     tl(1);
     asm volatile("s_waitcnt vmcnt(0)" ::: "memory");
     if (ADF_RB_FILL2) {
-        if (W3) issue_w(dc.w + (unsigned)(1 / NH) * slab + (unsigned)(1 % NH) * (unsigned)kPpWStage, 1);
+        if (W3) issue_w(slab_of(dc, 1), 1);
         issue_a01(d1, (unsigned)kPpAStage); issue_a23(d1, (unsigned)kPpAStage); issue_halo(d1, (unsigned)kPpAStage);
     }
     __syncthreads();
@@ -673,6 +681,7 @@
     const std::integral_constant<int, 0> c0{};
     const std::integral_constant<int, 1> c1{};
     const std::integral_constant<int, 2> c2{};
+    const std::integral_constant<int, 3> c3{};
     auto lds_barrier = [&]() __attribute__((always_inline)) { asm volatile("s_waitcnt lgkmcnt(0)\n\ts_barrier" ::: "memory"); };
     auto rotate = [&]() __attribute__((always_inline)) {
         const unsigned t = sa; sa = sa1; sa1 = sa2; sa2 = t;
@@ -683,12 +692,6 @@
     bool prev_one = false;
     int remaining = ntiles * nb;
 
-    auto next_slab = [&](int u, int taps_) __attribute__((always_inline)) -> const char* {
-        return dc.w + (unsigned)(u / NH) * slab + (unsigned)(u % NH) * (unsigned)kPpWStage;
-    };
-    auto slab_of = [&](const Blk& d, int v) __attribute__((always_inline)) -> const char* {
-        return d.w + (unsigned)(v / NH) * slab + (unsigned)(v % NH) * (unsigned)kPpWStage;
-    };
     auto issue_ahead = [&](int v, int ucur, bool has1, bool has2) __attribute__((always_inline)) -> int {
         if (v < ucur) { issue_w_at(slab_of(dc, v), ws2); return 2; }
         v -= ucur;
@@ -723,9 +726,13 @@
     int epi_vm = 0;
     bool slab1_pre = false;
     int aq_prev = 0;
-    auto block3 = [&](auto wpc) __attribute__((always_inline)) {
+    auto block3 = [&](auto wpc, auto tapsc, auto phc) __attribute__((always_inline)) {
         constexpr int WP = decltype(wpc)::value;
-        constexpr int U = 3 * NH;
+        constexpr int TAPS = decltype(tapsc)::value;
+        constexpr bool PH = decltype(phc)::value != 0;
+        static_assert(TAPS == 3 || (RAW && TAPS == 2), "a block with a prologue behind it has three sub-steps per N half");
+        static_assert(!PH || (RAW && NH == 2 && TAPS == 2), "the phase sub-steps: raw 256-column tiles");
+        constexpr int U = TAPS * NH;
 #ifdef ADF_RB_STAMP
         const bool stamp_on = bidx == 0 && tseq == 1 && kb == 2 && WP == 0;
         auto stamp = [&](int id) __attribute__((always_inline)) {
@@ -743,7 +750,7 @@
         stamp(0);
         rb_static_for<0, U>([&](auto uc) __attribute__((always_inline)) {
             constexpr int u = decltype(uc)::value;
-            constexpr int TAP = u / NH, HF = u % NH;
+            constexpr int TAP = PH ? (u + 1) / 2 : u / NH, HF = PH ? u / 2 : u % NH;
             const std::integral_constant<int, TAP> tapc{};
             const std::integral_constant<int, (WP + u) & 1> wstc{};
             const std::integral_constant<int, HF> hfc{};
@@ -753,10 +760,10 @@
                     [&](int ks) __attribute__((always_inline)) {
                         if (ks == 0) {
                             if (W3) wq = issue_ahead(u + 2, U, has1, has2);
-                            else if (u + 1 < U) { if (!(u == 0 && slab1_pre)) issue_w(next_slab(u + 1, 3), (WP + u + 1) & 1); }
+                            else if (u + 1 < U) { if (!(u == 0 && slab1_pre)) issue_w(slab_of(dc, u + 1), (WP + u + 1) & 1); }
                             else if (has1) issue_w(d1.w, (WP + u + 1) & 1);
                         } else if (ks == 1 && has2) {
-                            if (u == 0) { issue_halo(d2, sa2); issue_a01(d2, sa2); aq = (wave == 0 && d2.taps == 3) ? 3 : 2; }
+                            if (u == 0) { issue_halo(d2, sa2); issue_a01(d2, sa2); aq = (wave == 0 && d2.taps > 1) ? 3 : 2; }
                             else if (u == 1 && MH == 2) { issue_a23(d2, sa2); aq = 2; }
                         }
                     });
@@ -803,12 +810,12 @@
                     [&](int ks) __attribute__((always_inline)) {
                         if (ks == 0) {
                             if (W3) wq = issue_ahead(u + 2, NH, has1, has2);
-                            else if (u + 1 < NH) issue_w(next_slab(u + 1, 1), (WP + u + 1) & 1);
+                            else if (u + 1 < NH) issue_w(slab_of(dc, u + 1), (WP + u + 1) & 1);
                             else if (has1) issue_w(d1.w, (WP + u + 1) & 1);
                         } else if (u == NH - 1 && has2) {
                             if (ks == 1) { issue_a01(d2, sa2); aq += 2; }
                             else if (ks == 2) { issue_a23(d2, sa2); if (MH == 2) aq += 2; }
-                            else { issue_halo(d2, sa2); if (wave == 0 && d2.taps == 3) aq += 1; }
+                            else { issue_halo(d2, sa2); if (wave == 0 && d2.taps > 1) aq += 1; }
                         }
                     });
             if (W3) {
@@ -818,8 +825,8 @@
                 if (u == NH - 1 && has1) transform_all(d1, sa1);
             } else if (u == NH - 1) {
                 if (has2) {
-                    if (MH == 2) { if (wave == 0 && d2.taps == 3) asm volatile("s_waitcnt vmcnt(5)" ::: "memory"); else asm volatile("s_waitcnt vmcnt(4)" ::: "memory"); }
-                    else { if (wave == 0 && d2.taps == 3) asm volatile("s_waitcnt vmcnt(3)" ::: "memory"); else asm volatile("s_waitcnt vmcnt(2)" ::: "memory"); }
+                    if (MH == 2) { if (wave == 0 && d2.taps > 1) asm volatile("s_waitcnt vmcnt(5)" ::: "memory"); else asm volatile("s_waitcnt vmcnt(4)" ::: "memory"); }
+                    else { if (wave == 0 && d2.taps > 1) asm volatile("s_waitcnt vmcnt(3)" ::: "memory"); else asm volatile("s_waitcnt vmcnt(2)" ::: "memory"); }
                 }
                 else asm volatile("s_waitcnt vmcnt(0)" ::: "memory");
                 if (has1) transform_all(d1, sa1);
@@ -843,7 +850,7 @@
 #endif
             if (ADF_RB_PRESLAB) {
                 if (prev_one) { asm volatile("s_waitcnt vmcnt(0)" ::: "memory"); aq_prev = 0; prev_one = false; }
-                if (!W3) { issue_w(next_slab(1, 3), 1); slab1_pre = true; }
+                if (!W3) { issue_w(slab_of(dc, 1), 1); slab1_pre = true; }
                 epi_vm = NH * 4 * MH * (H.res != nullptr ? 2 : 1) + (H.stats != nullptr ? 2 * NH : 0);
             }
             epilogue(tile_of(tseq - 1), cur_tile.n0, sa2);
@@ -851,14 +858,23 @@
 #ifdef ADF_RB_TL
         tl(4 + tseq * 26 + 1);
 #endif
-        for (kb = 0; kb < nb3; kb += 2) {
-            block3(c0); rotate(); --remaining; prev_one = false;
-            block3(std::integral_constant<int, kPar3>{}); rotate(); --remaining;
-        }
-        for (int k1 = 0; k1 < nb1; k1 += 2) {
-            block1(c0); rotate(); --remaining;
-            block1(std::integral_constant<int, kPar1>{}); rotate(); --remaining; prev_one = true;
-        }
+        if constexpr (phase2) {
+#pragma nounroll
+            for (kb = 0; kb < nb3; ++kb) { block3(c0, c2, c1); rotate(); --remaining; }
+        } else {
+            for (kb = 0; kb < nb3; kb += 2) {
+                block3(c0, c3, c0); rotate(); --remaining; prev_one = false;
+                block3(std::integral_constant<int, kPar3>{}, c3, c0); rotate(); --remaining;
+            }
+            if constexpr (RAW)
+#pragma nounroll
+                for (; kb < nbh; ++kb) { block3(c0, c2, c0); rotate(); --remaining; }
+        }
+        if constexpr (!RAW)
+            for (int k1 = 0; k1 < nb1; k1 += 2) {
+                block1(c0); rotate(); --remaining;
+                block1(std::integral_constant<int, kPar1>{}); rotate(); --remaining; prev_one = true;
+            }
     }
     {
         const Tile last = tile_of(ntiles - 1);
diff --git a/audiodiffuser_amd/csrc/adf_net_unet1d.hip b/audiodiffuser_amd/csrc/adf_net_unet1d.hip
--- a/audiodiffuser_amd/csrc/adf_net_unet1d.hip
+++ b/audiodiffuser_amd/csrc/adf_net_unet1d.hip
@@ -427,6 +427,7 @@
         xv.C = x.C * f; xv.L = x.L / f; xv.stats = nullptr;
         GemmArgs g = W.gemm_base(y, xv.L, y.L, d.down);
         g.seg[0] = Walker1d::seg_of(xv, nullptr, nullptr, 1.f, 0, km + 1, 1, -(km / 2), 1, d.down);
+        g.seg[0].tap2_zero_c = folded_tap2_zero_from(d.down.K, f, x.C);
         W.run_gemm(g, y, true);
         W.tap("down" + std::to_string(i) + ".conv", y);
         x = y;
diff --git a/include/audiodiffuser_amd.h b/include/audiodiffuser_amd.h
--- a/include/audiodiffuser_amd.h
+++ b/include/audiodiffuser_amd.h
@@ -140,6 +140,8 @@
 int adf_debug_tap_copy(adf_handle* h, const char* name, float* out_fp32, void* stream);
 int adf_debug_tap_stats(adf_handle* h, const char* name, double* out_host, int* groups, void* stream);
 int adf_debug_up_tile_plan(int cin, int cout, int f, int B, int L, int* tile_rows, int* items, int* rounds, int* dead_rows);
+int adf_debug_rb_block_plan(int K, int f, int C, int phase_c, int n, int B, int L, int min_tiles, int zskip, int* tile_rows, int* nh, int* nb3, int* nb2,
+                            int* phase2);
 int adf_debug_dyn_threshold(adf_handle* h, float* x_dev, int B, long long per_sample, float quantile, void* stream);
 int adf_debug_coef_rows(adf_handle* h, float* out_dev, int max_rows, int* n_rows, void* stream);
 int adf_debug_tap_count(adf_handle* h);
```

Measured after the change: 4.512 million audio-samples/s, median of 6. 1.0% higher.
